# TIXhjq/ML_Function

Measured on AMD Instinct MI355X. Metric: samples/sec fwd+bwd xDeepFM-CIN B=4096,F=39,K=16, higher is better.
Workload: dtype f32

## Files before the change

ml_function_amd/csrc/cin.hip:

```cpp
#include "cin_kernels.h"
#include "cin_tail.h"
#include "cin_launch.h"
#include "cin_qtail.h"
#include "cin_qsplit.h"
#include "cin_qmerge.h"

#include <stdlib.h>

namespace fil {

struct CinShape {
  int B, F, K, L;
  int H[kCinMaxL];
  int Hp(int l) const { return l == 0 ? F : H[l - 1]; }
  int HS(int l) const { return 128 * cdiv(H[l], 128); }
  int xps(int l) const { return l == 0 ? F : HS(l - 1); }
  long M() const { return (long)B * K; }
  int JT() const { return cin_jt_of(F); }
  int HSmax() const {
    int h = 0;
    for (int l = 0; l < L; ++l) h = std::max(h, HS(l));
    return h;
  }
};

static int check_shape(const char* fn, int B, int F, int K, int L, const int* H, CinShape& s) {
  if (B < 0 || F < 1 || K < 1 || L < 1 || H == nullptr) return fail(FIL_ERR_ARG, "%s: bad shape B=%d F=%d K=%d L=%d", fn, B, F, K, L);
  if (L > kCinMaxL) return fail(FIL_ERR_UNSUPPORTED, "%s: L=%d > %d", fn, L, kCinMaxL);
  if (F > kCinMaxFields) return fail(FIL_ERR_UNSUPPORTED, "%s: F=%d > %d fields", fn, F, kCinMaxFields);
  if ((long)B * K > (1L << 28)) return fail(FIL_ERR_UNSUPPORTED, "%s: B*K = %ld rows > 2^28 (row-split byte offsets of the dW kernel are 32-bit)", fn, (long)B * K);
  s.B = B; s.F = F; s.K = K; s.L = L;
  for (int l = 0; l < L; ++l) {
    if (H[l] < 1) return fail(FIL_ERR_ARG, "%s: H[%d]=%d", fn, l, H[l]);
    if (H[l] > kCinMaxH) return fail(FIL_ERR_UNSUPPORTED, "%s: H[%d]=%d > %d feature maps", fn, l, H[l], kCinMaxH);
    s.H[l] = H[l];
  }
  return FIL_OK;
}

static int chunks_of(int H) { return cdiv(H, 128); }
static int env_int(const char* name, int dflt) {
  const char* v = getenv(name);
  return v != nullptr && *v != 0 ? atoi(v) : dflt;
}
struct Knobs {
  int mb, sym, dw_mb, dw_splits, dz_mb, tail_splits, tail_settle, tail_dz_mode, ksplit, dzs_mb, qtail, qmerge, dz2, fwdq, headfold, packfold, dwfold4;
};
static const Knobs& knobs() {
  static const Knobs k = {env_int("FIL_CIN_MB", 0), env_int("FIL_CIN_SYM", 1), env_int("FIL_CIN_DW_MB", 1), env_int("FIL_CIN_DW_SPLITS", 0),
                          env_int("FIL_CIN_DZ_MB", 1), env_int("FIL_CIN_TAIL_SPLITS", 0), env_int("FIL_CIN_TAIL_SETTLE", 0), env_int("FIL_CIN_TAIL_DZ_MODE", 0), env_int("FIL_CIN_KSPLIT", -1), env_int("FIL_CIN_DZS_MB", 0), env_int("FIL_CIN_QTAIL", 1), env_int("FIL_CIN_QMERGE", 1), env_int("FIL_CIN_DZ2", 1), env_int("FIL_CIN_FWDQ", 1), env_int("FIL_CIN_HEADFOLD", 1), env_int("FIL_CIN_PACKFOLD", 1), env_int("FIL_CIN_DWFOLD4", 1)};
  return k;
}
struct CinTune {
  int mb_forced;
  bool sym, no_ksplit;
  explicit CinTune(int mode)
      : mb_forced((mode & FIL_CIN_MB2) ? 2 : knobs().mb), sym(knobs().sym != 0 && !(mode & FIL_CIN_NOSYM)), no_ksplit((mode & FIL_CIN_NOKSPLIT) != 0) {}
  int mb_rows(long M) const {
    if (mb_forced == 1 || mb_forced == 2) return mb_forced;
    return cdiv((int)std::min<long>(M, 1L << 30), 64) >= 768 ? 2 : 1;
  }
  int ksplit(long M) const {
    if (knobs().ksplit == 0 || no_ksplit) return 1;
    if (mb_rows(M) != 1) return 1;
    if (knobs().ksplit == 4) return 4;
    return cdiv((int)std::min<long>(M, 1L << 30), 32) <= 512 ? 4 : 1;
  }
};

static const char* kFwdNames[kCinMaxL] = {"cin_fwd_l1", "cin_fwd_l2", "cin_fwd_l3", "cin_fwd_l4", "cin_fwd_l5", "cin_fwd_l6", "cin_fwd_l7", "cin_fwd_l8"};
static const char* kDwNames[kCinMaxL] = {"cin_bwd_dw_l1", "cin_bwd_dw_l2", "cin_bwd_dw_l3", "cin_bwd_dw_l4", "cin_bwd_dw_l5", "cin_bwd_dw_l6", "cin_bwd_dw_l7", "cin_bwd_dw_l8"};
static const char* kDzNames[kCinMaxL] = {"cin_bwd_dz_l1", "cin_bwd_dz_l2", "cin_bwd_dz_l3", "cin_bwd_dz_l4", "cin_bwd_dz_l5", "cin_bwd_dz_l6", "cin_bwd_dz_l7", "cin_bwd_dz_l8"};
static double gemm_flops(long M, int Hp, int F, int H) { return 2.0 * (double)M * Hp * F * H; }

struct DwPlan {
  int MB, blocks_x, splits, rows_per_split, chunks;
};
static int cu_count() {
  static const int n = [] {
    int dev = 0, v = 0;
    if (hipGetDevice(&dev) != hipSuccess || hipDeviceGetAttribute(&v, hipDeviceAttributeMultiprocessorCount, dev) != hipSuccess || v <= 0) v = 256;
    return v;
  }();
  return n;
}

static DwPlan dw_plan(long M, int C, int H) {
  DwPlan p;
  p.chunks = chunks_of(H);
  p.MB = knobs().dw_mb == 2 ? 2 : 1;
  const int waves_c = cdiv(C, 32 * p.MB);
  p.blocks_x = cdiv(waves_c, 4);
  const long tiles = (long)p.blocks_x * p.chunks;
  const long ncu = cu_count();
  const long unit = 2 * kDwDepth;
  auto rows_of = [&](int splits) { return std::max<long>(unit, ((M + splits - 1) / splits + unit - 1) / unit * unit); };
  int best = knobs().dw_splits;
  if (best <= 0) {
    static const double t_of[4] = {0.0, 1.05e-4, 1.39e-4, 1.96e-4};
    double best_ms = -1.0;
    for (int sp = (int)std::max<long>(1, (M + (1L << 20) - 1) >> 20); sp <= 256; ++sp) {
      const long rps = rows_of(sp);
      const long real = (M + rps - 1) / rps;
      if (real != sp && sp > 1) continue;
      long wgs = tiles * real;
      double per_row = 0.0;
      while (wgs > 0) {
        const long round = std::min(wgs, 3 * ncu);
        per_row += t_of[std::min<long>(3, (round + ncu - 1) / ncu)];
        wgs -= round;
      }
      const double ms = (double)rps * per_row * p.MB + (double)real * C * H * 4.0 / 6e9;
      if (best_ms < 0 || ms < best_ms) best = sp, best_ms = ms;
      if (rps == unit) break;
    }
  }
  best = std::min(std::max(best, 1), 256);
  const long rps = rows_of(best);
  p.rows_per_split = (int)rps;
  p.splits = (int)std::max<long>(1, (M + rps - 1) / rps);
  return p;
}

static int launch_dw3(hipStream_t st, const DwPlan& p, const float* gT, int HS, const float* xT, const float* xpT, int xps, float* part,
                      long M, int F, int Hp, int H, int symD = 0, int xtra = 0) {
  const int items = p.blocks_x * p.splits * p.chunks;
  const dim3 grid((items + 7) / 8 * 8);
#define FIL_DW3(MBV, ONES) \
  hipLaunchKernelGGL((cin_dw3_kernel<MBV, ONES>), grid, dim3(kCinThreads), 0, st, gT, HS, xT, xpT, xps, part, (int)M, F, Hp, H, p.rows_per_split, \
                     p.blocks_x, p.chunks, items, symD, xtra)
  if (xT == nullptr) {
    if (p.MB == 2) FIL_DW3(2, true); else FIL_DW3(1, true);
  } else {
    if (p.MB == 2) FIL_DW3(2, false); else FIL_DW3(1, false);
  }
#undef FIL_DW3
  return p.splits;
}

struct TailGeom {
  bool on = false;
  int p = 0;
  int NCB = 0, JP = 0, JT4 = 0, NQ = 0, JHp = 0;
  int Hpp = 0, Hq = 0, HL = 0, Cp = 0, C1 = 0;
  int periods = 0, tiles = 0;
  size_t uf_floats = 0, uz_floats = 0;
};
static TailGeom tail_geom(const CinShape& s) {
  TailGeom g;
  if (s.L < 3 || !cin_tail_supported(s.F)) return g;
  g.on = true;
  g.p = s.L - 2;
  g.NCB = cin_tail_ncb(s.F);
  g.JP = 16 * g.NCB;
  g.JT4 = cin_tail_jt4(s.F);
  g.NQ = cin_tail_nq(s.F);
  g.JHp = 4 * g.NQ;
  g.Hpp = s.H[g.p - 1];
  g.Hq = s.H[g.p];
  g.HL = s.H[s.L - 1];
  g.Cp = g.Hpp * s.F;
  g.C1 = g.Cp + 1;
  const int JT = s.JT();
  g.periods = cdiv(g.Hpp, cin_dz_h_per_period(JT));
  g.tiles = g.periods * cin_dz_tiles_per_period(JT) + 1;
  g.uf_floats = (size_t)g.Hpp * g.JT4 * 64 * g.NCB + (size_t)align_up(g.JP + 1, 64);
  g.uz_floats = (size_t)g.tiles * 64 * g.JHp;
  return g;
}
constexpr int kCinRetiredBits = 0;
static bool tail_used(const CinShape& s, int mode) {
  if ((mode & (FIL_CIN_GENERAL | FIL_CIN_NOTAIL)) != 0) return false;
  const TailGeom g = tail_geom(s);
  if (!g.on) return false;
  return (mode & FIL_CIN_TAIL_ALWAYS) != 0 || 4 * g.JP <= 3 * g.Hq;
}
static bool qtail_used(const CinShape& s, int mode, const CinTune& tune) {
  if (s.M() <= 16384 && (mode & FIL_CIN_TAIL_ALWAYS) == 0) return false;
  return tail_used(s, mode) && s.L == 3 && tune.sym && s.F >= 2 && s.F + 2 <= kQtConst && s.H[0] <= 128 && 3 * s.F + 1 <= s.HSmax() && (mode & FIL_CIN_NOQTAIL) == 0 &&
         knobs().qtail != 0;
}
static bool qmerge_used(const CinShape& s, int mode, const CinTune& tune) {
  return qtail_used(s, mode, tune) && 3 * s.F + 3 <= s.HSmax() && (mode & FIL_CIN_NOQMERGE) == 0 && knobs().qmerge != 0;
}
constexpr int kCinPrecBf16 = 1 << 20;
static int qsplit_planes(int mode) { return (mode & kCinPrecBf16) != 0 ? 1 : 3; }
static bool qsplit_fwd_menu(int JT) { return JT >= 2 && JT <= 12 && JT % 2 == 0; }
static bool qsplit_used(const CinShape& s, int mode, const CinTune& tune) {
  return (mode & (FIL_CIN_BF16X3 | kCinPrecBf16)) != 0 && qmerge_used(s, mode, tune) && knobs().fwdq != 0 && knobs().dz2 != 0 && s.HS(0) == 128 &&
         qsplit_fwd_menu(cin_jt_sym(s.F));
}
static size_t qsplit_wb_bytes(const CinShape& s) { return (size_t)cin_qs_steps(s.F, cin_jt_sym(s.F)) * kQsStageBytes; }
static size_t qsplit_wzb_bytes(const CinShape& s) {
  const int jts = cin_jt_sym(s.F);
  return ((size_t)cdiv(s.F, cin_dz_h_per_period(jts)) * cin_dz_tiles_per_period(jts) + 1) * 8 * 3072;
}
static size_t qtail_wz_floats(const CinShape& s) {
  const int jts = cin_jt_sym(s.F);
  return ((size_t)cdiv(s.F, cin_dz_h_per_period(jts)) * cin_dz_tiles_per_period(jts) + 1) * 32 * s.HS(0);
}
static size_t qtail_wsn_floats(const CinShape& s) { return (size_t)chunks_of(s.H[0]) * 2 * s.JT() * 128; }
static size_t qtail_saved_floats(const CinShape& s) {
  return (size_t)s.M() * s.HS(0) + (size_t)s.F * s.F * s.H[0] + (size_t)s.H[1] * s.F + 128 + (size_t)s.H[0] * s.F + qtail_wsn_floats(s) +
         qtail_wz_floats(s);
}
struct TailDwPlan {
  int blocks_x, splits, rows_per_split;
};
static TailDwPlan tail_dw_plan(long M, int C1) {
  TailDwPlan p;
  p.blocks_x = cdiv(C1, 16 * kTailCbw);
  const long unit = 4L * 4 * kTailDwDepth;
  long want = knobs().tail_splits > 0 ? knobs().tail_splits : std::max<long>(1, 2L * cu_count() / p.blocks_x);
  want = std::max<long>(want, (M + (1L << 22) - 1) >> 22);
  const long rows = std::max(unit, ((M + want - 1) / want + unit - 1) / unit * unit);
  p.rows_per_split = (int)rows;
  p.splits = (int)std::max<long>(1, (M + rows - 1) / rows);
  return p;
}

constexpr int kHeadChunk = 16;
constexpr int kColRows = 128;

static size_t saved_bytes(const CinShape& s) {
  size_t t = align_up((size_t)s.M() * s.F * sizeof(float), 256);
  for (int l = 0; l + 1 < s.L; ++l) t += align_up((size_t)s.M() * s.HS(l) * sizeof(float), 256);
  const TailGeom g = tail_geom(s);
  if (g.on) {
    size_t u = align_up((size_t)s.M() * s.F * sizeof(float), 256);
    for (int l = 0; l < g.p; ++l) u += align_up((size_t)s.M() * s.HS(l) * sizeof(float), 256);
    u += align_up((size_t)s.M() * g.JP * sizeof(float), 256) + align_up((g.uz_floats + g.uf_floats) * sizeof(float), 256) +
         align_up((size_t)g.Hq * s.F * sizeof(float), 256);
    t = std::max(t, u);
  }
  if (g.on && s.L == 3) {
    const size_t u = align_up((size_t)s.M() * s.F * sizeof(float), 256) + align_up((size_t)s.M() * s.HS(0) * sizeof(float), 256) +
                     align_up(qtail_saved_floats(s) * sizeof(float), 256);
    t = std::max(t, u);
  }
  return t;
}
static size_t wf_floats(const CinShape& s) {
  size_t w = 0;
  for (int l = 0; l < s.L; ++l) {
    w = std::max(w, (size_t)chunks_of(s.H[l]) * s.Hp(l) * 2 * s.JT() * 128);
  }
  w = std::max(w, (size_t)chunks_of(s.H[0]) * s.F * 2 * cin_jt_sym(s.F) * 128);
  w += (size_t)2 * 2 * s.JT() * 128;
  return w;
}
static int dz_periods(const CinShape& s, int l) { return cdiv(s.Hp(l), cin_dz_h_per_period(s.JT())); }
static size_t wz_floats(const CinShape& s) {
  const int jts = cin_jt_sym(s.F);
  size_t w = ((size_t)cdiv(s.F, cin_dz_h_per_period(jts)) * cin_dz_tiles_per_period(jts) + 1) * 32 * s.HS(0);
  w = std::max(w, (size_t)s.F * (s.F / 2 + 1) * s.H[0]);
  for (int l = 0; l < s.L; ++l) w = std::max(w, ((size_t)dz_periods(s, l) * cin_dz_tiles_per_period(s.JT()) + 1) * 32 * s.HS(l));
  return w;
}
static int pool_chunks(const CinShape& s, int l) { return std::max(chunks_of(s.H[l]), l > 0 ? chunks_of(s.H[l - 1]) : 1); }
static size_t fwd_ws_bytes(const CinShape& s) {
  size_t t = 0;
  for (int l = 0; l < s.L; ++l) t += align_up((size_t)pool_chunks(s, l) * s.M() * sizeof(float), 256);
  t += align_up((size_t)s.Hp(s.L - 1) * s.F * sizeof(float), 256);
  t += align_up(wf_floats(s) * sizeof(float), 256);
  t += align_up((size_t)kCinMaxH * sizeof(float), 256);
  t += align_up(cin_x2_floats(s.M(), cin_x2_len(s.F)) * sizeof(float), 256);
  t += align_up((size_t)chunks_of(s.H[0]) * s.F * 2 * cin_jt_sym(s.F) * 128 * sizeof(float), 256);
  t += align_up(qsplit_wb_bytes(s), 256);
  return t;
}
static size_t dw_part_floats(const CinShape& s) {
  size_t pmax = 0;
  for (int l = 0; l < s.L; ++l) pmax = std::max(pmax, (size_t)dw_plan(s.M(), s.Hp(l) * s.F, s.H[l]).splits * s.Hp(l) * s.F * s.H[l]);
  const int csym = s.F * (s.F / 2 + 1);
  pmax = std::max(pmax, (size_t)dw_plan(s.M(), csym, s.H[0]).splits * csym * s.H[0]);
  pmax = std::max(pmax, (size_t)dw_plan(s.M(), csym + s.F, s.H[0]).splits * (csym + s.F) * s.H[0]);
  if (s.L == 3) pmax = std::max(pmax, (size_t)cin_dwq_plan(s.M(), csym + s.F, cu_count()).pairs * (csym + s.F) * 256);
  if (s.L == 3) pmax = std::max(pmax, (size_t)cin_dwqb_plan(s.M(), csym + s.F, cu_count()).splits * (csym + s.F) * 256);
  pmax = std::max(pmax, (size_t)dw_plan(s.M(), s.Hp(s.L - 1), s.F).splits * s.Hp(s.L - 1) * s.F);
  pmax = std::max(pmax, (size_t)dw_plan(s.M(), s.F, s.Hp(s.L - 1)).splits * s.Hp(s.L - 1) * s.F);
  const TailGeom g = tail_geom(s);
  if (g.on) {
    pmax = std::max(pmax, (size_t)tail_dw_plan(s.M(), g.C1).splits * g.C1 * g.JP + (size_t)cdiv(g.Cp, kTailPc) * g.Hq * s.F);
  }
  return pmax;
}
static size_t bwd_ws_bytes(const CinShape& s) {
  const size_t LK = (size_t)s.L * s.K;
  const size_t M = (size_t)s.M();
  size_t t = 0;
  t += align_up((size_t)s.B * LK * sizeof(float), 256);
  t += 2 * align_up(M * s.HSmax() * sizeof(float), 256);
  t += align_up(dw_part_floats(s) * sizeof(float), 256);
  const size_t nblk = (size_t)cdiv(std::max(1, s.B), kHeadChunk);
  const size_t ncol = (M + kColRows - 1) / kColRows;
  t += align_up(std::max(ncol * s.HSmax(), nblk * (LK + 1)) * sizeof(float), 256);
  const size_t cl = (size_t)std::max(s.Hp(s.L - 1), s.L == 3 ? s.H[0] : 0) * s.F;
  t += 2 * align_up(cl * sizeof(float), 256);
  t += align_up(wz_floats(s) * sizeof(float), 256);
  t += 2 * align_up(M * s.F * sizeof(float), 256);
  t += align_up((size_t)s.F * s.F * kCinMaxH * sizeof(float), 256);
  t += align_up(((M + 255) / 256 + 1) * kQtConst * sizeof(float), 256);
  t += align_up(((M + 255) / 256) * (LK + 1) * sizeof(float), 256);
  t += 2 * align_up(qsplit_wzb_bytes(s), 256);
  return t;
}

template <typename KernelT>
static void allow_lds(KernelT kernel, size_t sh) {
  if (sh > 48 * 1024) (void)hipFuncSetAttribute(reinterpret_cast<const void*>(kernel), hipFuncAttributeMaxDynamicSharedMemorySize, (int)sh);
}

}

using namespace fil;

extern "C" size_t fil_cin_saved_bytes(int B, int F, int K, int L, const int* H) {
  CinShape s;
  if (check_shape("fil_cin_saved_bytes", B, F, K, L, H, s) != FIL_OK || B == 0) return 0;
  return saved_bytes(s);
}

extern "C" size_t fil_cin_fwd_workspace_bytes(int B, int F, int K, int L, const int* H) {
  CinShape s;
  if (check_shape("fil_cin_fwd_workspace_bytes", B, F, K, L, H, s) != FIL_OK || B == 0) return 0;
  return fwd_ws_bytes(s);
}

extern "C" size_t fil_cin_bwd_workspace_bytes(int B, int F, int K, int L, const int* H) {
  CinShape s;
  if (check_shape("fil_cin_bwd_workspace_bytes", B, F, K, L, H, s) != FIL_OK || B == 0) return 0;
  return bwd_ws_bytes(s);
}

extern "C" int fil_cin_grad_ready_points(int B, int F, int K, int L, const int* H, int mode, int* point) {
  CinShape s;
  if (int rc = check_shape("fil_cin_grad_ready_points", B, F, K, L, H, s)) return rc;
  if (point == nullptr || mode < 0 || mode > 1023) return fail(FIL_ERR_ARG, "fil_cin_grad_ready_points: point == NULL or mode %d out of range", mode);
  if ((mode & kCinRetiredBits) != 0) return fail(FIL_ERR_UNSUPPORTED, "fil_cin_grad_ready_points: mode %d holds a retired bit (2: the split-bf16 experiment)", mode);
  if (B == 0) {
    for (int i = 0; i <= L; ++i) point[i] = 0;
    return 1;
  }
  int pt = 0, l = L - 1;
  point[L] = pt++;
  if (qmerge_used(s, mode, CinTune(mode))) {
    point[0] = point[L] = 0;
    pt = 1;
    point[1] = point[2] = pt++;
    return pt;
  }
  if (tail_used(s, mode)) {
    point[L - 1] = point[L - 2] = pt++;
    l = L - 3;
  }
  for (; l >= 0; --l) point[l] = pt++;
  return pt;
}

#define FIL_CIN_CHECK_ARG(cond)                                                        \
  do {                                                                                 \
    if (!(cond)) return ::fil::fail(FIL_ERR_ARG, "%s: bad argument: %s", who, #cond); \
  } while (0)

static int cin_precision_bits(const char* who, int mode, int precision, int* bits) {
  if (precision != FIL_CIN_PREC_DEFAULT && precision != FIL_CIN_PREC_BF16)
    return fail(FIL_ERR_ARG, "%s: precision %d (0 DEFAULT, 1 BF16)", who, precision);
  if (precision == FIL_CIN_PREC_BF16 && (mode & FIL_CIN_BF16X3) != 0)
    return fail(FIL_ERR_ARG, "%s: precision BF16 with mode bit BF16X3 (mode %d): two operand precisions", who, mode);
  *bits = precision == FIL_CIN_PREC_BF16 ? kCinPrecBf16 : 0;
  return FIL_OK;
}

extern "C" int fil_cin_precision_used(int B, int F, int K, int L, const int* H, int mode, int precision) {
  CinShape s;
  if (int rc = check_shape("fil_cin_precision_used", B, F, K, L, H, s)) return rc;
  if (mode < 0 || mode > 1023 || (mode & kCinRetiredBits) != 0) return fail(FIL_ERR_UNSUPPORTED, "fil_cin_precision_used: mode %d", mode);
  int bits = 0;
  if (int rc = cin_precision_bits("fil_cin_precision_used", mode, precision, &bits)) return rc;
  if (bits == 0 || B == 0) return FIL_CIN_PREC_DEFAULT;
  return qsplit_used(s, mode | bits, CinTune(mode)) ? FIL_CIN_PREC_BF16 : FIL_CIN_PREC_DEFAULT;
}

static int cin_fwd_impl(const char* who, const float* x, const float* const* W, const float* const* bias, const float* dense_w,
                        const float* dense_b, float* out, float* pooled, float* saved, int B, int F, int K, int L,
                        const int* H, int output_dim, int mode, int precision, void* workspace, size_t workspace_bytes, void* stream) {
  CinShape s;
  int rc = check_shape(who, B, F, K, L, H, s);
  if (rc != FIL_OK) return rc;
  if (mode < 0 || mode > 1023 || (mode & kCinRetiredBits) != 0)
    return fail(FIL_ERR_UNSUPPORTED, "%s: mode %d (bits: 1 general kernels, 2 BF16X3, 4 MB2, 8 NOSYM, 16 X_TRANSPOSED, 32 NOTAIL, 64 TAIL_ALWAYS, 128 NOKSPLIT, 256 NOQTAIL, 512 NOQMERGE)", who, mode);
  {
    int bits = 0;
    if ((rc = cin_precision_bits(who, mode, precision, &bits)) != FIL_OK) return rc;
    mode |= bits;
  }
  const bool xt_in = (mode & FIL_CIN_X_TRANSPOSED) != 0;
  const CinTune tune(mode);
  const bool tail = tail_used(s, mode);
  const bool qtail = qtail_used(s, mode, tune);
  const bool qmerge = qmerge_used(s, mode, tune);
  const bool qsplit = qsplit_used(s, mode, tune);
  const int qnp = qsplit_planes(mode);
  const TailGeom tg = tail_geom(s);
  mode &= 1;
  if (B == 0) return FIL_OK;
  FIL_CIN_CHECK_ARG(x && W && bias && pooled && saved);
  FIL_CIN_CHECK_ARG(output_dim != 1 || (dense_w && dense_b && out));
  if (workspace == nullptr || workspace_bytes < fwd_ws_bytes(s))
    return fail(FIL_ERR_WORKSPACE, "fil_cin_fwd: workspace %zu < %zu bytes", workspace_bytes, fwd_ws_bytes(s));
  hipStream_t st = (hipStream_t)stream;
  const long M = s.M();
  const int JT = s.JT(), MB = tune.mb_rows(M);
  Carver ws(workspace);
  PoolArgs pa;
  for (int l = 0; l < L; ++l) {
    pa.part[l] = ws.take<float>((size_t)pool_chunks(s, l) * M);
    pa.chunks[l] = chunks_of(H[l]);
  }
  float* wsum = ws.take<float>((size_t)s.Hp(L - 1) * F);
  float* Wf = ws.take<float>(wf_floats(s));
  float* qt_zbias = ws.take<float>((size_t)kCinMaxH);
  const int XL = cin_x2_len(F);
  float* x2T = ws.take<float>(cin_x2_floats(M, XL));
  const bool need_x2 = tune.sym;
  float* WfT = ws.take<float>((size_t)chunks_of(H[0]) * F * 2 * cin_jt_sym(F) * 128);
  u32x4* Wb = reinterpret_cast<u32x4*>(ws.take<unsigned char>(qsplit_wb_bytes(s)));
  Carver sv(saved);
  float* xT_own = sv.take<float>((size_t)M * F);
  const float* xT = xt_in ? x : xT_own;
  float *tailY = nullptr, *tailUz = nullptr, *tailBmT = nullptr;
  float *qtR = nullptr, *qtT = nullptr, *qtWsumL = nullptr, *qtCvec = nullptr, *qtWsumP = nullptr, *qtWsnP = nullptr, *qtWzT = nullptr;
  if (qtail) {
    Carver pv(saved);
    (void)pv.take<float>((size_t)M * F);
    (void)pv.take<float>((size_t)M * s.HS(0));
    float* q = pv.take<float>(qtail_saved_floats(s));
    qtR = q;
    qtT = qtR + (size_t)M * s.HS(0);
    qtWsumL = qtT + (size_t)F * F * H[0];
    qtCvec = qtWsumL + (size_t)H[1] * F;
    qtWsumP = qtCvec + 128;
    qtWsnP = qtWsumP + (size_t)H[0] * F;
    qtWzT = qtWsnP + qtail_wsn_floats(s);
  } else if (tail) {
    Carver pv(saved);
    (void)pv.take<float>((size_t)M * F);
    for (int l = 0; l < tg.p; ++l) (void)pv.take<float>((size_t)M * s.HS(l));
    tailY = pv.take<float>((size_t)M * tg.JP);
    tailUz = pv.take<float>(tg.uz_floats + tg.uf_floats);
    tailBmT = pv.take<float>((size_t)tg.Hq * F);
  }
  const bool prep_fused = tail && tune.sym;
  if (qtail) {
    FIL_CIN_CHECK_ARG(W[0] && W[L - 1] && W[L - 2]);
    ProfScope ps("cin_fwd_prep", st, 2.0 * M * F * sizeof(float));
    const int JTs = cin_jt_sym(F), chunks0 = chunks_of(H[0]);
    const long npack = (long)chunks0 * F * 2 * JTs * 128;
    const bool fq = qmerge && knobs().fwdq != 0 && s.HS(0) == 128;
    const int nt = fq ? 0 : B, npk = (int)std::min<long>((npack + 255) / 256, 1024), nwl = cdiv(tg.Hq * F, 8), nwp = cdiv(tg.Hpp * F, 8);
    const size_t sh = (xt_in || fq) ? 0 : (size_t)F * (K + 1) * sizeof(float);
    allow_lds(cin_qtail_prep_kernel, sh);
    hipLaunchKernelGGL(cin_qtail_prep_kernel, dim3(nt + npk + nwl + nwp), dim3(256), sh, st, x, xT_own, F, K, nt, W[0], Wf, H[0], 2 * JTs, chunks0, npk,
                       W[L - 1], qtWsumL, tg.Hq, tg.HL, nwl, W[L - 2], qtWsumP, qtWsnP, tg.Hpp, 2 * JT, chunks_of(tg.Hpp), x2T, XL, xt_in ? 1 : 0);
  } else if (prep_fused) {
    FIL_CIN_CHECK_ARG(W[0] && W[L - 1]);
    ProfScope ps("cin_fwd_prep", st, 2.0 * M * F * sizeof(float));
    const int JTs = cin_jt_sym(F), chunks0 = chunks_of(H[0]);
    const long npack = (long)chunks0 * F * 2 * JTs * 128;
    const int nt = B, npk = (int)std::min<long>((npack + 255) / 256, 1024), nws = cdiv(tg.Hq * F, 8), nz = 64;
    const size_t sh = xt_in ? 0 : (size_t)F * (K + 1) * sizeof(float);
    allow_lds(cin_fwd_prep_kernel, sh);
    hipLaunchKernelGGL(cin_fwd_prep_kernel, dim3(nt + npk + nws + nz), dim3(256), sh, st, x, xT_own, F, K, nt, W[0], Wf, H[0], 2 * JTs, chunks0,
                       npk, W[L - 1], tailBmT, tg.Hq, tg.HL, nws, reinterpret_cast<float4*>(tailUz), (long)((tg.uz_floats + tg.uf_floats) / 4), x2T, XL,
                       xt_in ? 1 : 0);
  } else if (!xt_in || need_x2) {
    ProfScope ps("cin_transpose_in", st, 2.0 * M * F * sizeof(float));
    hipLaunchKernelGGL(cin_transpose_in_kernel, dim3(B), dim3(256), xt_in ? 0 : (size_t)F * (K + 1) * sizeof(float), st, x, xT_own, F, K,
                       need_x2 ? x2T : nullptr, XL, xt_in ? 1 : 0);
  }
  FIL_CHECK_LAUNCH();
  const float* xpT = xT;
  bool fused_last = false;
  bool head_done = false;
  for (int l = 0; l < L; ++l) {
    FIL_CIN_CHECK_ARG(W[l] && bias[l]);
    if (qtail && qmerge && l == 0 && knobs().fwdq != 0 && s.HS(0) == 128) {
      const int p = tg.p, lL = L - 1, Hpp = tg.Hpp, Hq = tg.Hq, HS0 = s.HS(0);
      FIL_CIN_CHECK_ARG(W[p] && W[lL] && bias[p] && bias[lL]);
      const int JTs = cin_jt_sym(F), chunks = chunks_of(Hpp);
      float* x1T = sv.take<float>((size_t)M * HS0);
      {
        ProfScope ps("cin_tail_prep", st);
        int ks = -1;
        if (!xt_in && K <= 64 && (K & (K - 1)) == 0 && (reinterpret_cast<uintptr_t>(x) & 15) == 0)
          for (ks = 0; (1 << ks) < K;) ++ks;
        const size_t sh_x = ks >= 0 ? (size_t)(64 >> ks) * F * (K + 1) : (xt_in ? (size_t)64 * (F | 1) : (size_t)F * (K + 1));
        const int tiles = cdiv(F, cin_dz_h_per_period(JTs)) * cin_dz_tiles_per_period(JTs) + 1;
        const bool fold = !qsplit && knobs().packfold != 0;
        const QtPackFold pf = fold ? QtPackFold{WfT, qtWzT, JTs, chunks, HS0, tiles} : QtPackFold{nullptr, nullptr, 0, 0, 0, 0};
        const size_t sh = std::max(cin_qtail_t_lds_floats(F, Hq, fold), sh_x) * sizeof(float);
        allow_lds(cin_qtail_t_x_kernel, sh);
        const int nx = (ks >= 0 || xt_in) ? (int)((M + 63) / 64) : B, nT = cin_qtail_t_wgs(Hpp);
        hipLaunchKernelGGL(cin_qtail_t_x_kernel, dim3(nT + nx), dim3(256), sh, st, W[p], qtWsumL, bias[p], bias[lL], tg.HL, qtT, qtCvec, qt_zbias, Hpp, F, Hq,
                           nT, x, xT_own, K, x2T, XL, xt_in ? 1 : 0, ks, (ks >= 0 || xt_in) ? (long)M : 0L, pf);
        if (!fold) {
          const long npack = (long)chunks * F * 2 * JTs * 128;
          const int nbf = (int)std::min<long>((npack + 255) / 256, 1024), nbz = (int)std::min<long>(((long)tiles * 32 * HS0 + 255) / 256, 1024);
          const int NTq = qsplit ? cin_qs_steps(F, JTs) : 0, nbq = qsplit ? std::min(cdiv(NTq * 512, 256), 512) : 0;
          if (qnp == 1)
            hipLaunchKernelGGL(cin_qtail_pack_kernel<1>, dim3(nbf + nbz + nbq), dim3(256), 0, st, qtT, WfT, qtWzT, F, Hpp, JTs, chunks, nbf, HS0, tiles, nbz,
                               W[0], H[0], Wb, NTq);
          else
            hipLaunchKernelGGL(cin_qtail_pack_kernel<3>, dim3(nbf + nbz + nbq), dim3(256), 0, st, qtT, WfT, qtWzT, F, Hpp, JTs, chunks, nbf, HS0, tiles, nbz,
                               W[0], H[0], Wb, NTq);
        }
      }
      FIL_CHECK_LAUNCH();
      {
        const double algo = gemm_flops(M, F, F, H[0]) + gemm_flops(M, Hpp, F, Hq) + gemm_flops(M, Hq, F, tg.HL);
        ProfScope ps("cin_fwd_q", st, algo, gemm_flops(M, 1, F * (F / 2 + 1), H[0]) + gemm_flops(M, 1, F * (F / 2 + 1), Hpp));
        CinHeadFold hf{};
        if (K <= 32 && (K & (K - 1)) == 0 && knobs().headfold != 0) {
          int ks = 0;
          while ((1 << ks) < K) ++ks;
          hf = CinHeadFold{pooled, output_dim == 1 ? out : nullptr, dense_w, dense_b, ks, (int)(L * K), p * K, lL * K};
          head_done = true;
        }
        if (qsplit) {
          const int NT = cin_qs_steps(F, JTs);
          if (!cin_launch_fwdq_b(st, qnp, JTs, x2T, XL, Wb, NT, bias[0], qtWsnP, JT, qtCvec, x1T, qtR, HS0, const_cast<float*>(pa.part[0]),
                                 const_cast<float*>(pa.part[p]), const_cast<float*>(pa.part[lL]), (int)M, F, H[0], hf))
            return fail(FIL_ERR_UNSUPPORTED, "fil_cin_fwd: no split-bf16 forward kernel for JT=%d (F=%d)", JTs, F);
        } else if (!cin_launch_fwdq(st, JTs, x2T, XL, Wf, WfT, bias[0], qtWsnP, JT, qtCvec, x1T, qtR, HS0, const_cast<float*>(pa.part[0]),
                                    const_cast<float*>(pa.part[p]), const_cast<float*>(pa.part[lL]), (int)M, F, H[0], hf))
          return fail(FIL_ERR_UNSUPPORTED, "fil_cin_fwd: no merged forward kernel for JT=%d (F=%d)", JTs, F);
        pa.chunks[0] = pa.chunks[p] = pa.chunks[lL] = 1;
      }
      FIL_CHECK_LAUNCH();
      break;
    }
    if (qtail && l == tg.p) {
      const int lL = L - 1, Hpp = tg.Hpp, Hq = tg.Hq, HS0 = s.HS(0);
      FIL_CIN_CHECK_ARG(W[lL] && bias[lL]);
      const int JTs = cin_jt_sym(F), chunks = chunks_of(Hpp);
      {
        ProfScope ps("cin_tail_prep", st);
        const size_t sh = cin_qtail_t_lds_floats(F, Hq, false) * sizeof(float);
        allow_lds(cin_qtail_t_kernel, sh);
        hipLaunchKernelGGL(cin_qtail_t_kernel, dim3(cin_qtail_t_wgs(Hpp)), dim3(256), sh, st, W[l], qtWsumL, bias[l], bias[lL], tg.HL, qtT, qtCvec, qt_zbias, Hpp, F, Hq);
        const long npack = (long)chunks * F * 2 * JTs * 128;
        const int tiles = cdiv(F, cin_dz_h_per_period(JTs)) * cin_dz_tiles_per_period(JTs) + 1;
        const int nbf = (int)std::min<long>((npack + 255) / 256, 1024), nbz = (int)std::min<long>(((long)tiles * 32 * HS0 + 255) / 256, 1024);
        hipLaunchKernelGGL(cin_qtail_pack_kernel<3>, dim3(nbf + nbz), dim3(256), 0, st, qtT, Wf, qtWzT, F, Hpp, JTs, chunks, nbf, HS0, tiles);
      }
      FIL_CHECK_LAUNCH();
      {
        const double algo = gemm_flops(M, Hpp, F, Hq) + gemm_flops(M, Hq, F, tg.HL);
        ProfScope ps("cin_fwd_tail", st, algo, gemm_flops(M, 1, F * (F / 2 + 1), Hpp));
        const int ks = tune.ksplit(M);
        cin_launch_fwd3_sym(st, MB, JTs, dim3(ks == 4 ? cdiv((int)M, 32) : cdiv((int)M, 128 * MB), chunks), xT, x2T, XL, Wf, qt_zbias, qtR, HS0,
                            const_cast<float*>(pa.part[lL]), (int)M, F, Hpp, ks);
      }
      FIL_CHECK_LAUNCH();
      {
        ProfScope ps("cin_tail_pool", st);
        const float* wsn = qtWsnP;
        float* pp = const_cast<float*>(pa.part[l]);
        float* pL = const_cast<float*>(pa.part[lL]);
        const dim3 grid((int)((M + 127) / 128));
#define FIL_QP(JTV) \
  case JTV: hipLaunchKernelGGL((cin_qtail_pool2_kernel<JTV>), grid, dim3(256), 0, st, xT, xpT, s.xps(l), wsn, qtR, HS0, qtCvec, pp, pL, (int)M, F, Hpp); break;
        switch (JT) { FIL_QP(4) FIL_QP(8) FIL_QP(12) FIL_QP(16) FIL_QP(20) FIL_QP(24) FIL_QP(28) FIL_QP(32) }
#undef FIL_QP
        pa.chunks[l] = pa.chunks[lL] = 1;
      }
      FIL_CHECK_LAUNCH();
      break;
    }
    if (tail && l == tg.p) {
      const int lL = L - 1;
      FIL_CIN_CHECK_ARG(W[lL] && bias[lL]);
      float* Y = tailY;
      float* Uz = tailUz;
      float* bmT = tailBmT;
      float* Uf = Uz + tg.uz_floats;
      float* consts = Uf + (size_t)tg.Hpp * tg.JT4 * 64 * tg.NCB;
      {
        ProfScope ps("cin_tail_prep", st);
        if (!prep_fused) {
          hipLaunchKernelGGL(cin_tail_wsum_kernel, dim3(cdiv(tg.Hq * F, 8)), dim3(256), 0, st, W[lL], bmT, tg.Hq, F, tg.HL);
          (void)hipMemsetAsync(Uz, 0, (tg.uz_floats + tg.uf_floats) * sizeof(float), st);
        }
        const size_t sh = (size_t)(F + 1) * (((tg.Hq + 3) & ~3) + 4) * sizeof(float);
        allow_lds(cin_tail_ueff_kernel, sh);
        hipLaunchKernelGGL(cin_tail_ueff_kernel, dim3(cdiv(tg.C1, kTailUc)), dim3(256), sh, st, W[l], bias[l], bmT, bias[lL], tg.HL, Uf, Uz, consts,
                           tg.Hpp, F, tg.Hq, tg.JT4, tg.JP, JT, tg.JHp);
      }
      FIL_CHECK_LAUNCH();
      {
        const double algo = gemm_flops(M, tg.Hpp, F, tg.Hq) + gemm_flops(M, tg.Hq, F, tg.HL);
        ProfScope ps("cin_fwd_tail", st, algo, 2.0 * (double)M * tg.Cp * (F + 1));
        const int RB = tune.mb_rows(M) == 2 ? 4 : 2;
        TailFwdArgs a{xT, xpT, s.xps(l), Uf, consts, Y, tg.JP, const_cast<float*>(pa.part[l]), const_cast<float*>(pa.part[lL]), (int)M, F, tg.Hpp,
                      tune.ksplit(M)};
        cin_launch_tail_fwd(st, RB, tg.JT4, tg.NCB, a);
        pa.chunks[l] = pa.chunks[lL] = 1;
      }
      FIL_CHECK_LAUNCH();
      break;
    }
    const int Hp = s.Hp(l), Hl = H[l], xps = s.xps(l);
    float* xoutT = l + 1 < L ? sv.take<float>((size_t)M * s.HS(l)) : nullptr;
    float* part = const_cast<float*>(pa.part[l]);
    const bool fuse_next = mode == 0 && l == L - 2 && !(l == 0 && tune.sym);
    if (l == L - 1 && mode == 0) {
      if (!fused_last) {
        const size_t sh = (size_t)Hp * ((F + 3) & ~3) * sizeof(float);
        ProfScope ps("cin_last_fwd", st, 2.0 * (double)M * Hp * F);
        hipLaunchKernelGGL(cin_wsum_kernel, dim3(cdiv(Hp * F, 8)), dim3(256), 0, st, W[l], wsum, Hp * F, Hl);
        allow_lds(cin_last_fwd_kernel, sh);
        hipLaunchKernelGGL(cin_last_fwd_kernel, dim3(cdiv((int)M, kLastRows)), dim3(256), sh, st, xT, xpT, xps, wsum, bias[l], part, (int)M, F, Hp, Hl);
        pa.chunks[l] = 1;
      }
    } else {
      const int chunks = chunks_of(Hl);
      if (l == 0 && tune.sym) {
        const int JTs = cin_jt_sym(F);
        const long npack = (long)chunks * F * 2 * JTs * 128;
        if (!prep_fused)
          hipLaunchKernelGGL(cin_pack_wf_sym_kernel, dim3((int)std::min<long>((npack + 255) / 256, 2048)), dim3(256), 0, st, W[l], Wf, F, Hl, 2 * JTs, chunks);
        ProfScope ps(kFwdNames[l], st, gemm_flops(M, Hp, F, Hl), gemm_flops(M, 1, F * (F / 2 + 1), Hl));
        const int ks = tune.ksplit(M);
        cin_launch_fwd3_sym(st, MB, JTs, dim3(ks == 4 ? cdiv((int)M, 32) : cdiv((int)M, 128 * MB), chunks), xT, x2T, XL, Wf, bias[l], xoutT, s.HS(l), part,
                            (int)M, F, Hl, ks);
      } else {
        const long npack = (long)chunks * Hp * 2 * JT * 128;
        hipLaunchKernelGGL(cin_pack_wf_kernel, dim3((int)std::min<long>((npack + 255) / 256, 2048)), dim3(256), 0, st, W[l], Wf, Hp, F, Hl, 2 * JT, chunks);
        const float* wsn = nullptr;
        if (fuse_next) {
          FIL_CIN_CHECK_ARG(W[l + 1] && bias[l + 1]);
          float* wsn_buf = Wf + (size_t)npack;
          hipLaunchKernelGGL(cin_wsum_wsn_kernel, dim3(cdiv(Hl * F, 8)), dim3(256), 0, st, W[l + 1], wsum, Hl * F, H[l + 1], wsn_buf, Hl, F, 2 * JT,
                             chunks);
          wsn = wsn_buf;
          pa.chunks[l + 1] = chunks;
          fused_last = true;
        }
        ProfScope ps(kFwdNames[l], st, gemm_flops(M, Hp, F, Hl) + (fuse_next ? 2.0 * (double)M * Hl * F : 0.0));
        cin_launch_fwd3(st, MB, JT, dim3(cdiv((int)M, 128 * MB), chunks), xT, xpT, xps, Wf, bias[l], xoutT, s.HS(l), part, (int)M, F, Hp, Hl,
                        wsn, fuse_next ? bias[l + 1] : nullptr, fuse_next ? H[l + 1] : 0, fuse_next ? const_cast<float*>(pa.part[l + 1]) : nullptr);
      }
    }
    FIL_CHECK_LAUNCH();
    xpT = xoutT;
  }
  if (!head_done) {
    ProfScope ps("cin_head_fwd", st);
    hipLaunchKernelGGL(cin_head_fwd_kernel, dim3(cdiv(B, kHeadSamples)), dim3(256), (size_t)kHeadSamples * L * K * sizeof(float), st, pa, dense_w, dense_b, pooled,
                       output_dim == 1 ? out : nullptr, B, K, L);
  }
  FIL_CHECK_LAUNCH();
  return FIL_OK;
}

extern "C" int fil_cin_fwd(const float* x, const float* const* W, const float* const* bias, const float* dense_w,
                           const float* dense_b, float* out, float* pooled, float* saved, int B, int F, int K, int L,
                           const int* H, int output_dim, int mode, void* workspace, size_t workspace_bytes, void* stream) {
  return cin_fwd_impl("fil_cin_fwd", x, W, bias, dense_w, dense_b, out, pooled, saved, B, F, K, L, H, output_dim, mode, FIL_CIN_PREC_DEFAULT, workspace,
                      workspace_bytes, stream);
}

extern "C" int fil_cin_fwd_p(const float* x, const float* const* W, const float* const* bias, const float* dense_w,
                             const float* dense_b, float* out, float* pooled, float* saved, int B, int F, int K, int L,
                             const int* H, int output_dim, int mode, int precision, void* workspace, size_t workspace_bytes, void* stream) {
  return cin_fwd_impl("fil_cin_fwd_p", x, W, bias, dense_w, dense_b, out, pooled, saved, B, F, K, L, H, output_dim, mode, precision, workspace,
                      workspace_bytes, stream);
}

static int cin_bwd_impl(const char* who, const float* x, const float* const* W, const float* const* bias, const float* dense_w,
                        const float* pooled, const float* saved, const float* g, float* dx, float* const* dW,
                        float* const* dbias, float* ddense_w, float* ddense_b, int B, int F, int K, int L, const int* H,
                        int output_dim, int mode, int precision, void* const* grad_ready_events, void* workspace, size_t workspace_bytes,
                        void* stream) {
  CinShape s;
  int rc = check_shape(who, B, F, K, L, H, s);
  if (rc != FIL_OK) return rc;
  if (mode < 0 || mode > 1023 || (mode & kCinRetiredBits) != 0)
    return fail(FIL_ERR_UNSUPPORTED, "%s: mode %d (bits: 1 general kernels, 2 BF16X3, 4 MB2, 8 NOSYM, 16 X_TRANSPOSED, 32 NOTAIL, 64 TAIL_ALWAYS, 128 NOKSPLIT, 256 NOQTAIL, 512 NOQMERGE)", who, mode);
  {
    int bits = 0;
    if ((rc = cin_precision_bits(who, mode, precision, &bits)) != FIL_OK) return rc;
    mode |= bits;
  }
  const bool xt_in = (mode & FIL_CIN_X_TRANSPOSED) != 0;
  const CinTune tune(mode);
  const bool tail = tail_used(s, mode);
  const bool qtail = qtail_used(s, mode, tune);
  const bool qmerge = qmerge_used(s, mode, tune);
  const bool qsplit = qsplit_used(s, mode, tune);
  const int qnp = qsplit_planes(mode);
  const TailGeom tg = tail_geom(s);
  mode &= 1;
  FIL_CIN_CHECK_ARG(W && dW && dbias);
  hipStream_t st = (hipStream_t)stream;
  const size_t LK = (size_t)L * K;
  auto ready = [&](int slot) {
    if (grad_ready_events != nullptr && grad_ready_events[slot] != nullptr) (void)hipEventRecord((hipEvent_t)grad_ready_events[slot], st);
  };
  if (B == 0) {
    for (int l = 0; l < L; ++l) {
      (void)hipMemsetAsync(dW[l], 0, (size_t)s.Hp(l) * F * H[l] * sizeof(float), st);
      (void)hipMemsetAsync(dbias[l], 0, (size_t)H[l] * sizeof(float), st);
    }
    if (output_dim == 1) {
      (void)hipMemsetAsync(ddense_w, 0, LK * sizeof(float), st);
      (void)hipMemsetAsync(ddense_b, 0, sizeof(float), st);
    }
    for (int l = 0; l <= L; ++l) ready(l);
    return FIL_OK;
  }
  FIL_CIN_CHECK_ARG(g && dx && saved && (x || !xt_in));
  FIL_CIN_CHECK_ARG(output_dim != 1 || (dense_w && pooled && ddense_w && ddense_b));
  if (workspace == nullptr || workspace_bytes < bwd_ws_bytes(s))
    return fail(FIL_ERR_WORKSPACE, "fil_cin_bwd: workspace %zu < %zu bytes", workspace_bytes, bwd_ws_bytes(s));
  const long M = s.M();
  const int JT = s.JT();
  Carver ws(workspace);
  float* dP = ws.take<float>((size_t)B * LK);
  float* Gbuf[2];
  Gbuf[0] = ws.take<float>((size_t)M * s.HSmax());
  Gbuf[1] = ws.take<float>((size_t)M * s.HSmax());
  float* part = ws.take<float>(dw_part_floats(s));
  const int nblk = cdiv(B, kHeadChunk);
  const int ncol = (int)((M + kColRows - 1) / kColRows);
  float* small = ws.take<float>(std::max((size_t)ncol * s.HSmax(), (size_t)nblk * (LK + 1)));
  const size_t cl = (size_t)s.Hp(L - 1) * F;
  const size_t cl_buf = (size_t)std::max(s.Hp(L - 1), L == 3 ? H[0] : 0) * F;
  float* wsum = ws.take<float>(cl_buf);
  float* vlast = ws.take<float>(cl_buf);
  float* Wz = ws.take<float>(wz_floats(s));
  float* dxT = ws.take<float>((size_t)M * F);
  float* gx0T = ws.take<float>((size_t)M * F);
  float* qt_dT = ws.take<float>((size_t)F * F * kCinMaxH);
  const int qt_ndc = (int)((M + 255) / 256);
  float* qt_dcpart = ws.take<float>((size_t)(qt_ndc + 1) * kQtConst);
  float* qt_hpart = ws.take<float>((size_t)qt_ndc * (LK + 1));
  u32x4* Wzb1 = reinterpret_cast<u32x4*>(ws.take<unsigned char>(qsplit_wzb_bytes(s)));
  u32x4* Wzb2 = reinterpret_cast<u32x4*>(ws.take<unsigned char>(qsplit_wzb_bytes(s)));

  Carver sv(const_cast<float*>(saved));
  const float* xT_own = sv.take<float>((size_t)M * F);
  const float* xT = xt_in ? x : xT_own;
  const float* maps[kCinMaxL];
  const float *tailY = nullptr, *tailUz = nullptr, *tailWsum = nullptr;
  const float *qtR = nullptr, *qtT = nullptr, *qtWsumL = nullptr, *qtCvec = nullptr, *qtWsumP = nullptr, *qtWsnP = nullptr, *qtWzT = nullptr;
  if (qtail) {
    maps[0] = sv.take<float>((size_t)M * s.HS(0));
    const float* q = sv.take<float>(qtail_saved_floats(s));
    qtR = q;
    qtT = qtR + (size_t)M * s.HS(0);
    qtWsumL = qtT + (size_t)F * F * H[0];
    qtCvec = qtWsumL + (size_t)H[1] * F;
    qtWsumP = qtCvec + 128;
    qtWsnP = qtWsumP + (size_t)H[0] * F;
    qtWzT = qtWsnP + qtail_wsn_floats(s);
  } else if (tail) {
    for (int l = 0; l < tg.p; ++l) maps[l] = sv.take<float>((size_t)M * s.HS(l));
    tailY = sv.take<float>((size_t)M * tg.JP);
    tailUz = sv.take<float>(tg.uz_floats + tg.uf_floats);
    tailWsum = sv.take<float>((size_t)tg.Hq * F);
  } else {
    for (int l = 0; l + 1 < L; ++l) maps[l] = sv.take<float>((size_t)M * s.HS(l));
  }

  const float* dPsrc = g;
  if (output_dim == 1 && qmerge) {
    dPsrc = dP;
  } else if (output_dim == 1) {
    ProfScope ps("cin_head_bwd", st);
    hipLaunchKernelGGL(cin_head_bwd_kernel, dim3(nblk), dim3(256), 0, st, g, dense_w, pooled, dP, small, B, (int)LK, kHeadChunk);
    if (!tail) hipLaunchKernelGGL(cin_reduce_kernel, dim3(cdiv((int)LK + 1, 64)), dim3(256), 0, st, small, ddense_w, (long)(LK + 1), nblk, ddense_b, (long)LK);
    FIL_CHECK_LAUNCH();
    dPsrc = dP;
  }
  if (!tail) ready(L);

  int cur = 0;
  int ltop = L - 1;
  bool dx_started = false;
  bool have_gx0 = false;
  bool wz_prepacked = false;
  bool qm_joined = false;
  if (qmerge) {
    const int p = tg.p, lL = L - 1, Hpp = tg.Hpp, Hq = tg.Hq, HS0 = s.HS(0);
    FIL_CIN_CHECK_ARG(bias && W[0] && W[p] && W[lL] && bias[p] && dW[0] && dW[p] && dW[lL] && dbias[0] && dbias[p] && dbias[lL]);
    const float* xpT = maps[p - 1];
    const int xps = s.xps(p);
    const float* dPp = dPsrc + (size_t)p * K;
    const float* dPL = dPsrc + (size_t)lL * K;
    const float* dPprev = dPsrc + (size_t)(p - 1) * K;
    const double algo_tail = gemm_flops(M, Hpp, F, Hq) + gemm_flops(M, Hq, F, tg.HL);
    const double algo1 = gemm_flops(M, F, F, H[0]);
    const int symD = F / 2 + 1, Cl = F * symD;
    const int JTs = cin_jt_sym(F);
    const int periods = cdiv(F, cin_dz_h_per_period(JTs));
    const int tiles0 = periods * cin_dz_tiles_per_period(JTs) + 1;
    const int XE = F + 3;
    float* xe = Gbuf[1];
    float* gxR = xe + (size_t)M * XE;
    float* dxR = gxR + (size_t)M * F;
    {
      ProfScope ps("cin_tail_a", st, (double)M * (2 * F + 3) * sizeof(float));
      const size_t sh = (size_t)256 * (F + 3 + (output_dim == 1 ? L : 0)) * sizeof(float);
      allow_lds(cin_qtail_xe_kernel<3>, sh);
      allow_lds(cin_qtail_xe_kernel<1>, sh);
      const int np = (int)std::min<long>(((long)tiles0 * 32 * HS0 + 255) / 256, 1024);
      const int nq2 = qsplit ? 2 * std::min(cdiv(tiles0 * 512, 256), 256) : 0;
      if (qnp == 1)
        hipLaunchKernelGGL(cin_qtail_xe_kernel<1>, dim3(qt_ndc + np + nq2), dim3(kXeThreads), sh, st, xT, dPL, dPp, (int)LK, K, xe, qt_dcpart, (int)M, F,
                           qt_ndc, output_dim == 1 ? g : nullptr, dense_w, pooled, dP, qt_hpart, (int)LK, lL, p, W[0], Wz, H[0], JTs, HS0, tiles0, np, qtT,
                           Hpp, Wzb1, Wzb2);
      else
        hipLaunchKernelGGL(cin_qtail_xe_kernel<3>, dim3(qt_ndc + np + nq2), dim3(kXeThreads), sh, st, xT, dPL, dPp, (int)LK, K, xe, qt_dcpart, (int)M, F,
                           qt_ndc, output_dim == 1 ? g : nullptr, dense_w, pooled, dP, qt_hpart, (int)LK, lL, p, W[0], Wz, H[0], JTs, HS0, tiles0, np, qtT,
                           Hpp, Wzb1, Wzb2);
    }
    FIL_CHECK_LAUNCH();
    {
      ProfScope ps("cin_last_bwd", st, 6.0 * (double)M * Hpp * F);
      cin_launch_last_bwd2(st, JT, xT, xpT, xps, qtWsumP, qtWsnP, dPp, (int)LK, dPprev, Gbuf[cur], HS0, dxT, (int)M, F, K, Hpp, qtR, HS0, dPL, small);
    }
    FIL_CHECK_LAUNCH();
    int dw_parts = 0;
    {
      ProfScope ps("cin_bwd_dw_q", st, algo1 + algo_tail, gemm_flops(M, 1, Cl, H[0]) + gemm_flops(M, 1, Cl, Hpp));
      if (qsplit) {
        const DwqbPlan bp = cin_dwqb_plan(M, Cl + F, cu_count());
        cin_launch_dwq_b(st, qnp, bp, Gbuf[cur], xpT, HS0, xe, XE, part, (int)M, F, symD);
        dw_parts = bp.splits;
      } else {
        const bool f4 = knobs().dwfold4 != 0;
        const DwqPlan dp = f4 ? cin_dwq_plan4(M, Cl + F, cu_count()) : cin_dwq_plan(M, Cl + F, cu_count());
        if (f4)
          hipLaunchKernelGGL((cin_dwq_kernel<kDwqDepth, 4>), dim3((dp.wgs + 7) / 8 * 8), dim3(kDwqThreads), 0, st, Gbuf[cur], xpT, HS0, xe, XE, part, (int)M, F,
                             symD, dp.rows_per_split, dp.splits, dp.ncol_full, dp.rem, dp.wgs_full, dp.wgs);
        else
          hipLaunchKernelGGL((cin_dwq_kernel<kDwqDepth, 2>), dim3((dp.wgs + 7) / 8 * 8), dim3(kDwqThreads), 0, st, Gbuf[cur], xpT, HS0, xe, XE, part, (int)M, F,
                             symD, dp.rows_per_split, dp.splits, dp.ncol_full, dp.rem, dp.wgs_full, dp.wgs);
        dw_parts = dp.pairs;
      }
    }
    FIL_CHECK_LAUNCH();
    {
      ProfScope ps("cin_reduce_dw", st);
      const int nb1 = cdiv(H[0], 64);
      const int nh = output_dim == 1 ? cdiv((int)LK + 1, 64) : 0;
      hipLaunchKernelGGL(cin_reduce_expand_q_kernel, dim3((Cl + F + 3) / 4 + nb1 + nh), dim3(256), 0, st, part, dw_parts, F, symD, H[0], Hpp, dW[0], qt_dT,
                         vlast, small, ncol, dbias[0], nb1, qt_hpart, qt_ndc, (int)LK, ddense_w, ddense_b);
    }
    FIL_CHECK_LAUNCH();
    ready(L);
    ready(0);
    {
      ProfScope ps("cin_tail_params", st);
      const size_t sh = cin_qtail_params_lds(F, Hq);
      allow_lds(cin_qtail_params_kernel, sh);
      float* dcfin = qt_dcpart + (size_t)qt_ndc * kQtConst;
      hipLaunchKernelGGL(cin_qtail_params_kernel, dim3(2 * Hpp + 1), dim3(256), sh, st, W[p], qtWsumL, qt_dT, vlast, dW[p], part, Hpp, F, Hq, qt_dcpart, qt_ndc,
                         dcfin);
      hipLaunchKernelGGL(cin_qtail_fill_kernel, dim3(cdiv(Hq * F, kQtFillCols)), dim3(kQtFillThreads), 0, st, part, Hpp, dcfin, bias[p], qtWsumL, dW[lL], dbias[p], dbias[lL], F, Hq,
                         tg.HL);
    }
    FIL_CHECK_LAUNCH();
    ready(lL);
    ready(p);
    const int NHMAX = HS0 / 2;
    if (NHMAX == 64 && knobs().dz2 != 0) {
      ProfScope ps("cin_bwd_dz_q", st, algo1 + algo_tail, gemm_flops(M, 1, Cl, H[0]) + gemm_flops(M, 1, Cl, Hpp));
      bool split_done = false;
      if (qsplit) {
        split_done = cin_launch_dz2_b(st, qnp, JTs, Gbuf[cur], xpT, HS0, dPL, (int)LK, K, Wzb1, Wzb2, xT, dxT, 1, (int)M, F, H[0], Hpp, periods, dx, qtCvec);
      }
      if (!split_done &&
          !cin_launch_dz2(st, JTs, Gbuf[cur], xpT, HS0, dPL, (int)LK, K, Wz, qtWzT, xT, dxT, 1, (int)M, F, H[0], Hpp, periods, dx, qtCvec))
        return fail(FIL_ERR_UNSUPPORTED, "fil_cin_bwd: no two-pass data-gradient kernel for JT=%d (F=%d)", JTs, F);
      qm_joined = true;
    } else {
      const bool two_waves = NHMAX == 64 && cin_dzs_two_waves(JTs) && tune.mb_forced != 2 && knobs().dzs_mb != 2;
      const int MBs = two_waves ? 1 : tune.mb_rows(M);
      const int ks = MBs != 1 ? 1 : tune.ksplit(M);
      const dim3 zgrid(ks == 4 ? cdiv((int)M, 32) : cdiv((int)M, 128 * MBs));
      {
        ProfScope ps("cin_bwd_dz_tail", st, algo_tail, gemm_flops(M, 1, Cl, Hpp));
        cin_launch_dz3_sym(st, MBs, JTs, NHMAX, zgrid, xpT, HS0, qtWzT, xT, gxR, dxR, 0, (int)M, F, Hpp, periods, ks);
      }
      FIL_CHECK_LAUNCH();
      {
        ProfScope ps("cin_bwd_dz_l1", st, algo1, gemm_flops(M, 1, Cl, H[0]));
        cin_launch_dz3_sym(st, MBs, JTs, NHMAX, zgrid, Gbuf[cur], HS0, Wz, xT, gx0T, dxT, 1, (int)M, F, H[0], periods, ks);
      }
      have_gx0 = true;
    }
    FIL_CHECK_LAUNCH();
    dx_started = true;
    ltop = -1;
  } else if (qtail) {
    const int p = tg.p, lL = L - 1, Hpp = tg.Hpp, Hq = tg.Hq, HS0 = s.HS(0);
    FIL_CIN_CHECK_ARG(bias && W[p] && W[lL] && bias[p] && dW[p] && dW[lL] && dbias[p] && dbias[lL]);
    const float* xpT = maps[p - 1];
    const int xps = s.xps(p);
    const float* dPp = dPsrc + (size_t)p * K;
    const float* dPL = dPsrc + (size_t)lL * K;
    const float* dPprev = dPsrc + (size_t)(p - 1) * K;
    const double algo = gemm_flops(M, Hpp, F, Hq) + gemm_flops(M, Hq, F, tg.HL);
    float* xs = Gbuf[1];
    float* gxR = xs + (size_t)M * (F + 1);
    float* dxR = gxR + (size_t)M * F;
    {
      ProfScope ps("cin_tail_a", st, (double)M * (F + 64) * sizeof(float));
      const size_t sh = (size_t)256 * (F + 3) * sizeof(float);
      allow_lds(cin_qtail_scale_kernel, sh);
      const int nh = output_dim == 1 ? cdiv((int)LK + 1, 64) : 0;
      FIL_CIN_CHECK_ARG(W[0]);
      const int JTs0 = cin_jt_sym(F);
      const int tiles0 = cdiv(F, cin_dz_h_per_period(JTs0)) * cin_dz_tiles_per_period(JTs0) + 1;
      const int np = (int)std::min<long>(((long)tiles0 * 32 * HS0 + 255) / 256, 1024);
      hipLaunchKernelGGL(cin_qtail_scale_kernel, dim3(qt_ndc + nh + np), dim3(256), sh, st, xT, dPL, dPp, (int)LK, K, xs, qt_dcpart, (int)M, F, qt_ndc, small,
                         ddense_w, ddense_b, (int)LK, nblk, nh, W[0], Wz, H[0], JTs0, HS0, tiles0);
      wz_prepacked = true;
    }
    FIL_CHECK_LAUNCH();
    ready(L);
    {
      ProfScope ps("cin_last_bwd", st, 6.0 * (double)M * Hpp * F);
      cin_launch_last_bwd2(st, JT, xT, xpT, xps, qtWsumP, qtWsnP, dPp, (int)LK, dPprev, Gbuf[cur], HS0, dxT, (int)M, F, K, Hpp, qtR, HS0, dPL, small);
    }
    FIL_CHECK_LAUNCH();
    const int symD = F / 2 + 1, Cl = F * symD;
    const int JTs = cin_jt_sym(F);
    {
      ProfScope ps("cin_bwd_dw_tail", st, algo, gemm_flops(M, 1, Cl, Hpp));
      const int parts = launch_dw3(st, dw_plan(M, Cl + F, Hpp), xpT, HS0, xT, xs, F + 1, part, M, F, F, Hpp, symD, F);
      const long nW = (long)Cl * Hpp, pstride = (long)(Cl + F) * Hpp;
      hipLaunchKernelGGL(cin_reduce_expand_sym_kernel, dim3((int)((nW + 63) / 64) + cdiv(F * Hpp, 64)), dim3(256), 0, st, part, qt_dT, F, symD, Hpp, parts,
                         pstride, vlast, (long)F * Hpp);
    }
    FIL_CHECK_LAUNCH();
    {
      ProfScope ps("cin_tail_params", st);
      const size_t sh = cin_qtail_params_lds(F, Hq);
      allow_lds(cin_qtail_params_kernel, sh);
      float* dcfin = qt_dcpart + (size_t)qt_ndc * kQtConst;
      hipLaunchKernelGGL(cin_qtail_params_kernel, dim3(2 * Hpp + 1), dim3(256), sh, st, W[p], qtWsumL, qt_dT, vlast, dW[p], part, Hpp, F, Hq, qt_dcpart, qt_ndc,
                         dcfin);
      hipLaunchKernelGGL(cin_qtail_fill_kernel, dim3(cdiv(Hq * F, kQtFillCols)), dim3(kQtFillThreads), 0, st, part, Hpp, dcfin, bias[p], qtWsumL, dW[lL], dbias[p], dbias[lL], F, Hq,
                         tg.HL);
    }
    FIL_CHECK_LAUNCH();
    ready(lL);
    ready(p);
    {
      const int periods = cdiv(F, cin_dz_h_per_period(JTs));
      ProfScope ps("cin_bwd_dz_tail", st, algo, gemm_flops(M, 1, Cl, Hpp));
      const int NHMAX = HS0 / 2;
      const bool two_waves = NHMAX == 64 && cin_dzs_two_waves(JTs) && tune.mb_forced != 2 && knobs().dzs_mb != 2;
      const int MBs = two_waves ? 1 : tune.mb_rows(M);
      const int ks = MBs != 1 ? 1 : tune.ksplit(M);
      cin_launch_dz3_sym(st, MBs, JTs, NHMAX, dim3(ks == 4 ? cdiv((int)M, 32) : cdiv((int)M, 128 * MBs)), xpT, HS0, qtWzT, xT, gxR, dxR, 0, (int)M, F, Hpp,
                         periods, ks);
    }
    FIL_CHECK_LAUNCH();
    dx_started = true;
    ltop = p - 1;
  } else if (tail) {
    const int p = tg.p, lL = L - 1;
    FIL_CIN_CHECK_ARG(bias && W[p] && W[lL] && bias[p] && dW[p] && dW[lL] && dbias[p] && dbias[lL]);
    const float* xpT = maps[p - 1];
    const int xps = s.xps(p);
    const double algo = gemm_flops(M, tg.Hpp, F, tg.Hq) + gemm_flops(M, tg.Hq, F, tg.HL);
    float* Apk = Gbuf[1];
    wz_prepacked = p == 1 && tune.sym && F >= 2;
    {
      ProfScope ps("cin_tail_a", st, (double)M * (F + 64) * sizeof(float));
      const int na = (int)std::min<long>((M * 16 * tg.NCB + 255) / 256, 4096);
      const int nh = output_dim == 1 ? cdiv((int)LK + 1, 64) : 0;
      int np = 0, JTs = 0, tiles0 = 0;
      if (wz_prepacked) {
        FIL_CIN_CHECK_ARG(W[0]);
        JTs = cin_jt_sym(F);
        tiles0 = cdiv(F, cin_dz_h_per_period(JTs)) * cin_dz_tiles_per_period(JTs) + 1;
        np = (int)std::min<long>(((long)tiles0 * 32 * s.HS(0) + 255) / 256, 1024);
      }
      hipLaunchKernelGGL(cin_tail_pre_kernel, dim3(na + nh + np), dim3(256), 0, st, xT, dPsrc, (int)LK, K, p, lL, Apk, (int)M, F, tg.NCB, na, small,
                         ddense_w, ddense_b, (int)LK, nblk, nh, W[0], Wz, H[0], JTs, s.HS(0), tiles0);
    }
    FIL_CHECK_LAUNCH();
    ready(L);
    const TailDwPlan tp = tail_dw_plan(M, tg.C1);
    {
      ProfScope ps("cin_bwd_dw_tail", st, algo, 2.0 * (double)M * tg.C1 * (F + 2));
      TailDwArgs a{Apk, xT, xpT, xps, part, (int)M, F, tg.Hpp, tg.JP, tp.rows_per_split, tp.blocks_x, tp.blocks_x * tp.splits, knobs().tail_settle != 0};
      cin_launch_tail_dw(st, tg.NCB, a);
    }
    FIL_CHECK_LAUNCH();
    {
      ProfScope ps("cin_tail_params", st);
      const int nblk_p = cdiv(tg.Cp, kTailPc);
      const int ldb = (tg.Hq + 3) & ~3;
      const size_t sh = ((size_t)(F + 1) * ldb + (size_t)tg.JP * (kTailPc + 4) + (size_t)kTailPc * ldb) * sizeof(float);
      allow_lds(cin_tail_params_kernel, sh);
      float* partB = part + (size_t)tp.splits * tg.C1 * tg.JP;
      float* qones = vlast;
      hipLaunchKernelGGL(cin_tail_params_kernel, dim3(2 * nblk_p), dim3(256), sh, st, part, tp.splits, W[p], tailWsum, dW[p], dbias[p], partB, qones,
                         tg.Cp, F, tg.Hq, tg.JP);
      hipLaunchKernelGGL(cin_tail_fill_kernel, dim3(cdiv(tg.Hq * F, 64)), dim3(256), 0, st, partB, nblk_p, qones, bias[p], dW[lL], dbias[lL], F,
                         tg.Hq, tg.HL);
    }
    FIL_CHECK_LAUNCH();
    ready(lL);
    ready(p);
    {
      ProfScope ps("cin_bwd_dz_tail", st, algo, 2.0 * (double)M * tg.Cp * (F + 1));
      TailDzArgs a{tailUz, xT, xpT, xps, tailY, tg.JP, dPsrc, (int)LK, K, p, lL, Gbuf[cur], s.HS(p - 1), dxT, (int)M, F, tg.Hpp, tg.periods, knobs().tail_dz_mode,
                   tune.ksplit(M)};
      cin_launch_tail_dz(st, JT, tg.NQ, a);
    }
    FIL_CHECK_LAUNCH();
    dx_started = true;
    ltop = p - 1;
  } else if (mode == 0) {
    const int l = L - 1;
    FIL_CIN_CHECK_ARG(W[l] && dW[l] && dbias[l]);
    const int Hp = s.Hp(l), Hl = H[l], xps = s.xps(l);
    const float* xpT = l == 0 ? xT : maps[l - 1];
    const float* dPl = dPsrc + (size_t)l * K;
    const float* dPprev = l > 0 ? dPsrc + (size_t)(l - 1) * K : nullptr;
    const size_t shw = (size_t)Hp * ((F + 3) & ~3) * sizeof(float);
    ProfScope ps("cin_last_bwd", st, 6.0 * (double)M * Hp * F);
    hipLaunchKernelGGL(cin_wsum_wsn_kernel, dim3(cdiv(Hp * F, 8)), dim3(256), 0, st, W[l], wsum, Hp * F, Hl, l > 0 ? Wz : nullptr, Hp, F, 2 * JT,
                       chunks_of(Hp));
    hipLaunchKernelGGL(cin_slice_sum_kernel, dim3(nblk), dim3(256), 0, st, dPl, (int)LK, small, B, K, kHeadChunk);
    {
      float* yT = Gbuf[1];
      const int YS = (F + 3) & ~3;
      const long tot = M * YS;
      hipLaunchKernelGGL(cin_scale_rows3_kernel, dim3((int)std::min<long>((tot + 255) / 256, 4096)), dim3(256), 0, st, xT, dPl, (int)LK, K, yT, (int)M, F, YS);
      const bool swap = l > 0;
      int nb;
      if (swap) nb = launch_dw3(st, dw_plan(M, F, Hp), xpT, xps, nullptr, yT, YS, part, M, 1, F, Hp);
      else nb = launch_dw3(st, dw_plan(M, Hp, F), yT, YS, nullptr, xpT, xps, part, M, 1, Hp, F);
      hipLaunchKernelGGL(cin_reduce_kernel, dim3(cdiv((int)cl, 64)), dim3(256), 0, st, part, vlast, (long)cl, nb);
      hipLaunchKernelGGL(cin_fill_rows_kernel, dim3((int)std::min<long>(((long)cl * Hl + 255) / 256, 2048)), dim3(256), 0, st, vlast, dW[l], (long)cl, Hl,
                         swap ? F : 0, Hp, small, nblk, dbias[l]);
    }
    ready(l);
    if (l > 0) {
      cin_launch_last_bwd2(st, JT, xT, xpT, xps, wsum, Wz, dPl, (int)LK, dPprev, Gbuf[cur], s.HS(l - 1), dxT, (int)M, F, K, Hp);
    } else {
      const size_t shb = shw + (size_t)kLastRows * (kLastFMax + 1) * sizeof(float);
      allow_lds(cin_last_bwd_kernel, shb);
      hipLaunchKernelGGL(cin_last_bwd_kernel, dim3(cdiv((int)M, kLastRows)), dim3(256), shb, st, xT, xpT, xps, wsum, dPl, (int)LK, dPprev,
                         nullptr, 0, dxT, 1, (int)M, F, K, Hp);
    }
    FIL_CHECK_LAUNCH();
    dx_started = true;
    ltop = L - 2;
  } else {
    const long total = M * s.HS(L - 1);
    ProfScope ps("cin_bcast_g", st, (double)total * sizeof(float));
    hipLaunchKernelGGL(cin_bcast3_kernel, dim3((int)std::min<long>((total + 255) / 256, 4096)), dim3(256), 0, st, dPsrc + (size_t)(L - 1) * K, (int)LK,
                       K, Gbuf[cur], s.HS(L - 1), (int)M, H[L - 1]);
    FIL_CHECK_LAUNCH();
  }
  for (int l = ltop; l >= 0; --l) {
    FIL_CIN_CHECK_ARG(W[l] && dW[l] && dbias[l]);
    const int Hp = s.Hp(l), Hl = H[l], HSl = s.HS(l), xps = s.xps(l);
    const float* xpT = l == 0 ? xT : maps[l - 1];
    const float* G = Gbuf[cur];
    {
      ProfScope ps("cin_dbias", st, (double)M * Hl * sizeof(float));
      if (!(qtail && l == ltop)) hipLaunchKernelGGL(cin_colsum3_kernel, dim3(ncol), dim3(256), 0, st, G, HSl, small, (int)M, Hl, kColRows);
      hipLaunchKernelGGL(cin_reduce_kernel, dim3(cdiv(Hl, 64)), dim3(256), 0, st, small, dbias[l], (long)Hl, ncol);
    }
    FIL_CHECK_LAUNCH();
    int parts;
    const int symD = (l == 0 && tune.sym) ? F / 2 + 1 : 0;
    const int Cl = symD > 0 ? F * symD : Hp * F;
    {
      ProfScope ps(kDwNames[l], st, gemm_flops(M, Hp, F, Hl), gemm_flops(M, 1, Cl, Hl));
      parts = launch_dw3(st, dw_plan(M, Cl, Hl), G, HSl, xT, xpT, xps, part, M, F, Hp, Hl, symD);
    }
    FIL_CHECK_LAUNCH();
    const long nW = (long)Cl * Hl;
    {
      ProfScope ps("cin_reduce_dw", st, (double)(parts + 1) * nW * sizeof(float));
      if (symD > 0) hipLaunchKernelGGL(cin_reduce_expand_sym_kernel, dim3((int)((nW + 63) / 64)), dim3(256), 0, st, part, dW[l], F, symD, Hl, parts);
      else hipLaunchKernelGGL(cin_reduce_kernel, dim3((int)((nW + 63) / 64)), dim3(256), 0, st, part, dW[l], nW, parts);
    }
    FIL_CHECK_LAUNCH();
    ready(l);
    {
      const int NHMAX = HSl / 2;
      const int MB = NHMAX == 128 ? 1 : tune.mb_rows(M);
      const int MBg = NHMAX == 128 ? 1 : ((knobs().dz_mb == 2 && JT <= 28) ? 2 : 1);
      const float* dPprev = l > 0 ? dPsrc + (size_t)(l - 1) * K : nullptr;
      if (l == 0 && tune.sym && F >= 2) {
        const int JTs = cin_jt_sym(F);
        const int periods = cdiv(F, cin_dz_h_per_period(JTs));
        const int tiles = periods * cin_dz_tiles_per_period(JTs) + 1;
        const long npack = (long)tiles * 32 * HSl;
        const bool two_waves = NHMAX == 64 && cin_dzs_two_waves(JTs) && tune.mb_forced != 2 && knobs().dzs_mb != 2;
        const int MBs = two_waves ? 1 : MB;
        if (!wz_prepacked) {
          hipLaunchKernelGGL(cin_pack_wz_sym_kernel, dim3((int)std::min<long>((npack + 255) / 256, 2048)), dim3(256), 0, st, W[l], Wz, F, Hl, JTs, HSl, tiles);
        }
        ProfScope ps(kDzNames[l], st, gemm_flops(M, Hp, F, Hl), gemm_flops(M, 1, F * (F / 2 + 1), Hl));
        const int ks = (NHMAX != 64 || MBs != 1) ? 1 : tune.ksplit(M);
        cin_launch_dz3_sym(st, MBs, JTs, NHMAX, dim3(ks == 4 ? cdiv((int)M, 32) : cdiv((int)M, 128 * MBs)), G, HSl, Wz, xT, gx0T, dxT,
                           dx_started ? 1 : 0, (int)M, F, Hl, periods, ks);
      } else {
        const int periods = dz_periods(s, l);
        const int tiles = periods * cin_dz_tiles_per_period(JT) + 1;
        const long npack = (long)tiles * 32 * HSl;
        hipLaunchKernelGGL(cin_pack_wz_kernel, dim3((int)std::min<long>((npack + 255) / 256, 2048)), dim3(256), 0, st, W[l], Wz, Hp, F, Hl, JT, HSl, tiles);
        ProfScope ps(kDzNames[l], st, gemm_flops(M, Hp, F, Hl));
        cin_launch_dz3(st, MBg, JT, NHMAX, dim3(cdiv((int)M, 128 * MBg)), G, HSl, Wz, xT, xpT, xps, dPprev, (int)LK, K,
                       l > 0 ? Gbuf[cur ^ 1] : nullptr, l > 0 ? s.HS(l - 1) : 0, l == 0 ? gx0T : nullptr, dxT, dx_started ? 1 : 0,
                       (int)M, F, Hp, Hl, periods);
      }
      dx_started = true;
      if (l == 0) have_gx0 = true;
    }
    FIL_CHECK_LAUNCH();
    cur ^= 1;
  }
  if (!qm_joined) {
    ProfScope ps("cin_transpose_out", st, 2.0 * M * F * sizeof(float));
    if (qmerge)
      hipLaunchKernelGGL(cin_transpose_out_kernel, dim3(B), dim3(256), (size_t)K * (F + 1) * sizeof(float), st, dxT, have_gx0 ? gx0T : nullptr, dx, F, K,
                         Gbuf[1] + (size_t)M * (F + 3), Gbuf[1] + (size_t)M * (F + 3) + (size_t)M * F, qtCvec, dPsrc + (size_t)(L - 1) * K, (int)LK);
    else if (qtail)
      hipLaunchKernelGGL(cin_transpose_out_kernel, dim3(B), dim3(256), (size_t)K * (F + 1) * sizeof(float), st, dxT, have_gx0 ? gx0T : nullptr, dx, F, K,
                         Gbuf[1] + (size_t)M * (F + 1), Gbuf[1] + (size_t)M * (F + 1) + (size_t)M * F, qtCvec, dPsrc + (size_t)(L - 1) * K, (int)LK);
    else
      hipLaunchKernelGGL(cin_transpose_out_kernel, dim3(B), dim3(256), (size_t)K * (F + 1) * sizeof(float), st, dxT, have_gx0 ? gx0T : nullptr, dx, F, K);
  }
  FIL_CHECK_LAUNCH();
  return FIL_OK;
}

extern "C" int fil_cin_bwd(const float* x, const float* const* W, const float* const* bias, const float* dense_w,
                           const float* pooled, const float* saved, const float* g, float* dx, float* const* dW,
                           float* const* dbias, float* ddense_w, float* ddense_b, int B, int F, int K, int L, const int* H,
                           int output_dim, int mode, void* const* grad_ready_events, void* workspace, size_t workspace_bytes,
                           void* stream) {
  return cin_bwd_impl("fil_cin_bwd", x, W, bias, dense_w, pooled, saved, g, dx, dW, dbias, ddense_w, ddense_b, B, F, K, L, H, output_dim, mode,
                      FIL_CIN_PREC_DEFAULT, grad_ready_events, workspace, workspace_bytes, stream);
}

extern "C" int fil_cin_bwd_p(const float* x, const float* const* W, const float* const* bias, const float* dense_w,
                             const float* pooled, const float* saved, const float* g, float* dx, float* const* dW,
                             float* const* dbias, float* ddense_w, float* ddense_b, int B, int F, int K, int L, const int* H,
                             int output_dim, int mode, int precision, void* const* grad_ready_events, void* workspace, size_t workspace_bytes,
                             void* stream) {
  return cin_bwd_impl("fil_cin_bwd_p", x, W, bias, dense_w, pooled, saved, g, dx, dW, dbias, ddense_w, ddense_b, B, F, K, L, H, output_dim, mode,
                      precision, grad_ready_events, workspace, workspace_bytes, stream);
}
```

ml_function_amd/csrc/cin_kernels.h:

```cpp
#pragma once
#include "common.h"

namespace fil {

constexpr int kCinThreads = 256;
constexpr int kCinMaxL = 8;
constexpr int kCinMaxH = 256;

__device__ __forceinline__ f32x16 mfma32(float a, float b, f32x16 c) {
  return __builtin_amdgcn_mfma_f32_32x32x2f32(a, b, c, 0, 0, 0);
}

__device__ __forceinline__ void settle(float& v) { asm volatile("" : "+v"(v)); }
typedef float f32x4s __attribute__((ext_vector_type(4)));
__device__ __forceinline__ void settle(f32x4s& v) { asm volatile("" : "+v"(v)); }

__device__ __forceinline__ __amdgpu_buffer_rsrc_t make_rsrc(const float* p, long bytes) {
  return __builtin_amdgcn_make_buffer_rsrc(const_cast<float*>(p), 0, (int)std::min<long>(bytes, 0x7fffffffL), 0x00020000);
}
__device__ __forceinline__ __amdgpu_buffer_rsrc_t make_rsrc_uniform(const float* p, long bytes) {
  const unsigned long a = reinterpret_cast<unsigned long>(p);
  const unsigned lo = __builtin_amdgcn_readfirstlane((unsigned)a), hi = __builtin_amdgcn_readfirstlane((unsigned)(a >> 32));
  const int n = __builtin_amdgcn_readfirstlane((int)std::min<long>(bytes, 0x7fffffffL));
  return __builtin_amdgcn_make_buffer_rsrc(reinterpret_cast<float*>(((unsigned long)hi << 32) | lo), 0, n, 0x00020000);
// ... 956 lines not shown
  const long total = (long)M * YS;
  for (long i = (long)blockIdx.x * blockDim.x + threadIdx.x; i < total; i += (long)gridDim.x * blockDim.x) {
    const long m = i / YS;
    const int f = (int)(i - m * YS);
    const long b = m / K;
    yT[i] = f < F ? xT[m * F + f] * dP[b * ldp + (m - b * K)] : 0.f;
  }
}

__device__ __forceinline__ void cin_reduce_body(const float* __restrict__ part, float* __restrict__ out, long n, int parts,
                                                float* __restrict__ out2, long n1, int bid, long pstride = 0) {
  __shared__ float red[4][64];
  const int lane = threadIdx.x & 63, wave = threadIdx.x >> 6;
  const long i = (long)bid * 64 + lane;
  const long ps = pstride > 0 ? pstride : n;
  float t0 = 0.f, t1 = 0.f, t2 = 0.f, t3 = 0.f;
  if (i < n) {
    int p = wave;
    for (; p + 60 < parts; p += 64) {
      float u[16];
#pragma unroll
      for (int e = 0; e < 16; ++e) u[e] = part[(long)(p + 4 * e) * ps + i];
#pragma unroll
      for (int e = 0; e < 16; e += 4) {
        t0 += u[e];
        t1 += u[e + 1];
        t2 += u[e + 2];
        t3 += u[e + 3];
      }
    }
    for (; p + 12 < parts; p += 16) {
      t0 += part[(long)p * ps + i];
      t1 += part[(long)(p + 4) * ps + i];
      t2 += part[(long)(p + 8) * ps + i];
      t3 += part[(long)(p + 12) * ps + i];
    }
    for (; p < parts; p += 4) t0 += part[(long)p * ps + i];
  }
  red[wave][lane] = (t0 + t1) + (t2 + t3);
  __syncthreads();
  if (wave == 0 && i < n) {
    const float v = (red[0][lane] + red[1][lane]) + (red[2][lane] + red[3][lane]);
    if (out2 != nullptr && i >= n1) out2[i - n1] = v;
    else out[i] = v;
  }
}
static __global__ __launch_bounds__(256) void cin_reduce_kernel(const float* __restrict__ part, float* __restrict__ out, long n,
                                                         int parts, float* __restrict__ out2 = nullptr, long n1 = 0, long pstride = 0) {
  cin_reduce_body(part, out, n, parts, out2, n1, blockIdx.x, pstride);
}

static __global__ __launch_bounds__(256) void cin_reduce_expand_sym_kernel(const float* __restrict__ part, float* __restrict__ dW, int F, int D,
                                                                    int H, int parts, long pstride = 0, float* __restrict__ vout = nullptr,
                                                                    long nv = 0) {
  if (vout != nullptr) {
    const long nbw = ((long)F * D * H + 63) / 64;
    if ((long)blockIdx.x >= nbw) {
      cin_reduce_body(part + (long)F * D * H, vout, nv, parts, nullptr, 0, (int)(blockIdx.x - nbw), pstride);
      return;
    }
  }
  __shared__ float red[4][64];
  const int lane = threadIdx.x & 63, wave = threadIdx.x >> 6;
  const long n = (long)F * D * H;
  const long ps = pstride > 0 ? pstride : n;
  const long i = (long)blockIdx.x * 64 + lane;
  float t0 = 0.f, t1 = 0.f, t2 = 0.f, t3 = 0.f;
  if (i < n) {
    int p = wave;
    for (; p + 60 < parts; p += 64) {
      float u[16];
#pragma unroll
      for (int e = 0; e < 16; ++e) u[e] = part[(long)(p + 4 * e) * ps + i];
#pragma unroll
      for (int e = 0; e < 16; e += 4) {
        t0 += u[e];
        t1 += u[e + 1];
        t2 += u[e + 2];
        t3 += u[e + 3];
      }
    }
    for (; p + 12 < parts; p += 16) {
      t0 += part[(long)p * ps + i];
      t1 += part[(long)(p + 4) * ps + i];
      t2 += part[(long)(p + 8) * ps + i];
      t3 += part[(long)(p + 12) * ps + i];
    }
    for (; p < parts; p += 4) t0 += part[(long)p * ps + i];
  }
  red[wave][lane] = (t0 + t1) + (t2 + t3);
  __syncthreads();
  if (wave == 0 && i < n) {
    const float v = (red[0][lane] + red[1][lane]) + (red[2][lane] + red[3][lane]);
    const int col = (int)(i % H);
    const int pair = (int)(i / H);
    const int h = pair / D, d = pair - h * D;
    const int f = (h + d) % F;
    dW[((long)h * F + f) * H + col] = v;
    if (d != 0 && 2 * d != F) dW[((long)f * F + h) * H + col] = v;
  }
}

static __global__ __launch_bounds__(256) void cin_slice_sum_kernel(const float* __restrict__ dP, int ldp, float* __restrict__ part, int B,
                                                            int K, int bchunk) {
  __shared__ float red[256];
  const int b_lo = blockIdx.x * bchunk, b_hi = min(B, b_lo + bchunk);
  float t = 0.f;
  const int total = (b_hi - b_lo) * K;
  for (int i = threadIdx.x; i < total; i += 256) {
    const int b = b_lo + i / K, k = i % K;
    t += dP[(long)b * ldp + k];
  }
  red[threadIdx.x] = t;
  __syncthreads();
  for (int s = 128; s > 0; s >>= 1) {
    if (threadIdx.x < s) red[threadIdx.x] += red[threadIdx.x + s];
    __syncthreads();
  }
  if (threadIdx.x == 0) part[blockIdx.x] = red[0];
}

constexpr int kLastFMax = 64;

static __global__ __launch_bounds__(256) void cin_wsum_kernel(const float* __restrict__ W, float* __restrict__ wsum, int C, int H) {
  const int row = blockIdx.x * 8 + (threadIdx.x >> 5), l = threadIdx.x & 31;
  float t = 0.f;
  if (row < C)
    for (int n = l; n < H; n += 32) t += W[(long)row * H + n];
  t = half_wave_sum(t);
  if (row < C && l == 0) wsum[row] = t;
}

static __global__ __launch_bounds__(256) void cin_wsum_wsn_kernel(const float* __restrict__ W, float* __restrict__ wsum, int C, int H,
                                                           float* __restrict__ wsn, int Hp, int F, int JT2, int chunks) {
  const int row = blockIdx.x * 8 + (threadIdx.x >> 5), l = threadIdx.x & 31;
  float t = 0.f;
  if (row < C)
    for (int n = l; n < H; n += 32) t += W[(long)row * H + n];
  t = half_wave_sum(t);
  if (row < C && l == 0) {
    wsum[row] = t;
    if (wsn != nullptr) {
      const int n = row / F, fp = row - n * F;
      wsn[(((n >> 7) * JT2) + fp) * 128 + (n & 127)] = t;
    }
  }
  if (wsn != nullptr) {
    const int total = chunks * JT2 * 128;
    for (int i = blockIdx.x * blockDim.x + threadIdx.x; i < total; i += gridDim.x * blockDim.x) {
      const int col = i & 127, fp = (i >> 7) % JT2, chunk = (i >> 7) / JT2;
      if (fp >= F || chunk * 128 + col >= Hp) wsn[i] = 0.f;
    }
  }
}

__device__ __forceinline__ void stage_wsum(const float* __restrict__ wsum, float* ws, int Hp, int F, int FP4) {
  for (int idx = threadIdx.x; idx < Hp * FP4; idx += blockDim.x) {
    const int h = idx / FP4, f = idx - h * FP4;
    ws[idx] = f < F ? wsum[h * F + f] : 0.f;
  }
}

constexpr int kLastRows = 64;

static __global__ __launch_bounds__(256) void cin_last_fwd_kernel(const float* __restrict__ xT, const float* __restrict__ xpT, int xps,
                                                           const float* __restrict__ wsum, const float* __restrict__ bias,
                                                           float* __restrict__ pool, int M, int F, int Hp, int H) {
  extern __shared__ __attribute__((aligned(16))) float smem[];
  const int FP4 = (F + 3) & ~3;
  stage_wsum(wsum, smem, Hp, F, FP4);
  float bsum = 0.f;
  for (int n = 0; n < H; ++n) bsum += bias[n];
  __syncthreads();
  const int lane = threadIdx.x & 63, wave = threadIdx.x >> 6;
  const int m = blockIdx.x * kLastRows + wave * 16 + (lane & 15), hq = lane >> 4;
  const bool valid = m < M;
  const long mm = valid ? m : 0;
  float xr[kLastFMax];
#pragma unroll
  for (int f = 0; f < kLastFMax; ++f) xr[f] = (valid && f < F) ? xT[mm * F + f] : 0.f;
  const float* xprow = xpT + mm * xps;
  float p = 0.f;
  for (int h = hq; h < Hp; h += 4) {
    const float4* wrow = reinterpret_cast<const float4*>(smem + h * FP4);
    float t = 0.f;
#pragma unroll
    for (int f4 = 0; f4 < kLastFMax / 4; ++f4) {
      if (4 * f4 < F) {
        const float4 w = wrow[f4];
        t = fmaf(xr[4 * f4], w.x, t);
        t = fmaf(xr[4 * f4 + 1], w.y, t);
        t = fmaf(xr[4 * f4 + 2], w.z, t);
        t = fmaf(xr[4 * f4 + 3], w.w, t);
      }
    }
    p = fmaf(valid ? xprow[h] : 0.f, t, p);
  }
  p += __shfl_xor(p, 16);
  p += __shfl_xor(p, 32);
  if (valid && hq == 0) pool[m] = p + bsum;
}

static __global__ __launch_bounds__(256) void cin_last_bwd_kernel(const float* __restrict__ xT, const float* __restrict__ xpT, int xps,
                                                           const float* __restrict__ wsum, const float* __restrict__ dP, int ldp,
                                                           const float* __restrict__ dPprev, float* __restrict__ GprevT, int HSp,
                                                           float* __restrict__ dxT, int layer1, int M, int F, int K, int Hp) {
  extern __shared__ __attribute__((aligned(16))) float smem[];
  const int FP4 = (F + 3) & ~3;
  float* ts = smem + Hp * FP4;
  stage_wsum(wsum, smem, Hp, F, FP4);
  __syncthreads();
  const int lane = threadIdx.x & 63, wave = threadIdx.x >> 6;
  const int rowl = wave * 16 + (lane & 15), hq = lane >> 4;
  const int m = blockIdx.x * kLastRows + rowl;
  const bool valid = m < M;
  const long mm = valid ? m : 0;
  const int b = (int)(mm / K), k = (int)(mm - (long)b * K);
  float xr[kLastFMax], u[kLastFMax];
#pragma unroll
  for (int f = 0; f < kLastFMax; ++f) {
    xr[f] = (valid && f < F) ? xT[mm * F + f] : 0.f;
    u[f] = 0.f;
  }
  const float dp = valid ? dP[(long)b * ldp + k] : 0.f;
  const float dpp = (valid && dPprev != nullptr) ? dPprev[(long)b * ldp + k] : 0.f;
  const float* xprow = xpT + mm * xps;
  for (int h = hq; h < Hp; h += 4) {
    const float4* wrow = reinterpret_cast<const float4*>(smem + h * FP4);
    const float xph = valid ? xprow[h] : 0.f;
    float t = 0.f;
#pragma unroll
    for (int f4 = 0; f4 < kLastFMax / 4; ++f4) {
      if (4 * f4 < F) {
        const float4 w = wrow[f4];
        t = fmaf(xr[4 * f4], w.x, t);
        t = fmaf(xr[4 * f4 + 1], w.y, t);
        t = fmaf(xr[4 * f4 + 2], w.z, t);
        t = fmaf(xr[4 * f4 + 3], w.w, t);
        u[4 * f4] = fmaf(xph, w.x, u[4 * f4]);
        u[4 * f4 + 1] = fmaf(xph, w.y, u[4 * f4 + 1]);
        u[4 * f4 + 2] = fmaf(xph, w.z, u[4 * f4 + 2]);
        u[4 * f4 + 3] = fmaf(xph, w.w, u[4 * f4 + 3]);
      }
    }
    if (layer1) ts[rowl * (kLastFMax + 1) + h] = t;
    else if (valid) GprevT[mm * HSp + h] = fmaf(dp, t, dpp);
  }
  if (layer1) __syncthreads();
#pragma unroll
  for (int f = 0; f < kLastFMax; ++f) {
    if (f < F) {
      float v = u[f];
      v += __shfl_xor(v, 16);
      v += __shfl_xor(v, 32);
      if (layer1) v += ts[rowl * (kLastFMax + 1) + f];
      if (valid && hq == 0) dxT[mm * F + f] = dp * v;
    }
  }
}

static __global__ __launch_bounds__(256) void cin_fill_rows_kernel(const float* __restrict__ v, float* __restrict__ dW, long C, int H, int Ft,
                                                            int Hp, const float* __restrict__ bpart = nullptr, int bparts = 0,
                                                            float* __restrict__ dbias = nullptr) {
  if (bpart != nullptr && blockIdx.x == 0) {
    __shared__ float red[256];
    float t = 0.f;
    for (int p = threadIdx.x; p < bparts; p += 256) t += bpart[p];
    red[threadIdx.x] = t;
    __syncthreads();
    for (int s = 128; s > 0; s >>= 1) {
      if (threadIdx.x < s) red[threadIdx.x] += red[threadIdx.x + s];
      __syncthreads();
    }
    const float tot = red[0];
    for (int n = threadIdx.x; n < H; n += 256) dbias[n] = tot;
  }
  const long total = C * H;
  for (long i = (long)blockIdx.x * blockDim.x + threadIdx.x; i < total; i += (long)gridDim.x * blockDim.x) {
    const long c = i / H;
    dW[i] = Ft > 0 ? v[(c % Ft) * Hp + c / Ft] : v[c];
  }
}

constexpr int kLast2Ld = 66;
constexpr int kLast2Stage = 32 * kLast2Ld;
template <int JT>
__global__ __launch_bounds__(256, 2) void cin_last_bwd2_kernel(const float* __restrict__ xT, const float* __restrict__ xpT, int xps,
                                                            const float* __restrict__ wsum, const float* __restrict__ wsn,
                                                            const float* __restrict__ dP, int ldp, const float* __restrict__ dPprev,
                                                            float* __restrict__ GprevT, int HSp, float* __restrict__ dxT, int M, int F,
                                                            int K, int Hp, const float* __restrict__ Radd = nullptr, int HSr = 0,
                                                            const float* __restrict__ dPadd = nullptr, float* __restrict__ colpart = nullptr) {
  __shared__ float colred[4][128];
  extern __shared__ __attribute__((aligned(16))) float smem[];
  for (int i = threadIdx.x; i < Hp * F; i += 256) smem[i] = wsum[i];
  __syncthreads();
  const int tid = threadIdx.x, lane = tid & 63, wave = tid >> 6;
  const int r = lane & 31, half = lane >> 5;
  const int wrow0 = (blockIdx.x * 4 + wave) * 32;
  if (wrow0 >= M && colpart == nullptr) return;
  const long mq = min(wrow0 + r, M - 1);
  float* stg = smem + ((Hp * F + 3) & ~3) + wave * kLast2Stage;
  const int nrow = min(32, M - wrow0);
  if (nrow > 0) {
    const float4* src = reinterpret_cast<const float4*>(xT + (long)wrow0 * F);
    const int n4 = nrow * F / 4, tail = nrow * F - 4 * n4;
    for (int i = lane; i < n4; i += 64) *reinterpret_cast<float4*>(stg + 4 * i) = src[i];
    if (lane < tail) stg[4 * n4 + lane] = xT[(long)wrow0 * F + 4 * n4 + lane];
  }
  __builtin_amdgcn_wave_barrier();
  float xr[JT];
  {
    const float* xrow = stg + min(r, max(nrow, 1) - 1) * F;
#pragma unroll
    for (int j = 0; j < JT; ++j) {
      const int f = 2 * j + half;
      xr[j] = (f < F && nrow > 0) ? xrow[min(f, F - 1)] : 0.f;
    }
  }
  __shared__ float dps[4][3][32];
  if (half == 0) {
    const int b = (int)(mq / K), k = (int)(mq - (long)b * K);
    dps[wave][0][r] = dP[(long)b * ldp + k];
    dps[wave][1][r] = dPprev != nullptr ? dPprev[(long)b * ldp + k] : 0.f;
    dps[wave][2][r] = Radd != nullptr ? dPadd[(long)b * ldp + k] : 0.f;
  }
  __builtin_amdgcn_wave_barrier();
  auto phase_t = [&]() {
  const int chunks = (Hp + 127) >> 7;
  for (int chunk = 0; chunk < chunks; ++chunk) {
    f32x16 t[4];
#pragma unroll
    for (int nb = 0; nb < 4; ++nb)
#pragma unroll
      for (int i = 0; i < 16; ++i) t[nb][i] = 0.f;
    const float4* wsb = reinterpret_cast<const float4*>(wsn + (long)chunk * (2 * JT) * 128) + (half * 32 + r);
    constexpr int QB = JT % 5 == 0 ? 5 : 4;
#pragma unroll
    for (int j0 = 0; j0 < JT; j0 += QB) {
      float4 wq[QB];
#pragma unroll
      for (int j = 0; j < QB; ++j) wq[j] = wsb[(long)(2 * (j0 + j)) * 32];
      __builtin_amdgcn_sched_barrier(0);
#pragma unroll
      for (int j = 0; j < QB; ++j) {
        const float4 w = wq[j];
        t[0] = mfma32(xr[j0 + j], w.x, t[0]);
        t[1] = mfma32(xr[j0 + j], w.y, t[1]);
        t[2] = mfma32(xr[j0 + j], w.z, t[2]);
        t[3] = mfma32(xr[j0 + j], w.w, t[3]);
      }
    }
    const int n0 = chunk * 128 + 4 * r;
    float c0 = 0.f, c1 = 0.f, c2 = 0.f, c3 = 0.f;
    float4 rq[8];
#pragma unroll
    for (int reg = 0; reg < 16; ++reg) {
      if (Radd != nullptr && (reg & 7) == 0) {
#pragma unroll
        for (int u = 0; u < 8; ++u) {
          const long mm = min(wrow0 + mfma32_row(reg + u, half), M - 1);
          rq[u] = *reinterpret_cast<const float4*>(Radd + mm * HSr + n0);
        }
      }
      const int row = mfma32_row(reg, half);
      const int m = wrow0 + row;
      const float dpr = dps[wave][0][row], dppr = dps[wave][1][row], dpa = dps[wave][2][row];
      if (m < M) {
        float* dst = GprevT + (long)m * HSp + n0;
        float v0 = fmaf(dpr, t[0][reg], dppr), v1 = fmaf(dpr, t[1][reg], dppr);
        float v2 = fmaf(dpr, t[2][reg], dppr), v3 = fmaf(dpr, t[3][reg], dppr);
        if (Radd != nullptr) {
          const float4 ra = rq[reg & 7];
          v0 = fmaf(dpa, ra.x, v0);
          v1 = fmaf(dpa, ra.y, v1);
          v2 = fmaf(dpa, ra.z, v2);
          v3 = fmaf(dpa, ra.w, v3);
        }
        c0 += v0;
        c1 += v1;
        c2 += v2;
        c3 += v3;
        if (n0 + 3 < Hp) {
          *reinterpret_cast<float4*>(dst) = make_float4(v0, v1, v2, v3);
        } else {
          if (n0 < Hp) dst[0] = v0;
          if (n0 + 1 < Hp) dst[1] = v1;
          if (n0 + 2 < Hp) dst[2] = v2;
        }
      }
    }
    if (colpart != nullptr) {
      c0 = lane_halves_sum(c0);
      c1 = lane_halves_sum(c1);
      c2 = lane_halves_sum(c2);
      c3 = lane_halves_sum(c3);
      if (half == 0) *reinterpret_cast<float4*>(&colred[wave][4 * r]) = make_float4(c0, c1, c2, c3);
      __syncthreads();
      for (int n = tid; n < 128; n += 256)
        if (chunk * 128 + n < Hp) colpart[(long)blockIdx.x * Hp + chunk * 128 + n] = (colred[0][n] + colred[1][n]) + (colred[2][n] + colred[3][n]);
      __syncthreads();
    }
  }
  };
  auto phase_u = [&]() {
  if (wrow0 >= M) return;
  f32x16 u0, u1;
#pragma unroll
  for (int i = 0; i < 16; ++i) u0[i] = u1[i] = 0.f;
  const bool two = F > 32;
  const int quads = (Hp + 3) >> 2;
#pragma unroll 1
  for (int q0 = 0; q0 < quads; q0 += 16) {
    __builtin_amdgcn_wave_barrier();
    {
      float4 v[8];
#pragma unroll
      for (int i = 0; i < 8; ++i) {
        const int row = (lane >> 4) + 4 * i, c4 = lane & 15;
        const long mm = min(wrow0 + row, M - 1);
        v[i] = 4 * q0 + 4 * c4 < xps ? *reinterpret_cast<const float4*>(xpT + mm * xps + 4 * q0 + 4 * c4) : make_float4(0.f, 0.f, 0.f, 0.f);
      }
#pragma unroll
      for (int i = 0; i < 8; ++i) {
        const int row = (lane >> 4) + 4 * i, c4 = lane & 15;
        float* d = stg + row * kLast2Ld + 4 * c4;
        *reinterpret_cast<float2*>(d) = make_float2(v[i].x, v[i].y);
        *reinterpret_cast<float2*>(d + 2) = make_float2(v[i].z, v[i].w);
      }
    }
    __builtin_amdgcn_wave_barrier();
    float2 av[16];
    const float* xprow = stg + r * kLast2Ld + 2 * half;
#pragma unroll
    for (int i = 0; i < 16; ++i) av[i] = q0 + i < quads ? *reinterpret_cast<const float2*>(xprow + 4 * i) : make_float2(0.f, 0.f);
#pragma unroll
    for (int i0 = 0; i0 < 16; i0 += 4) {
      float b0[4][2], b1[4][2];
#pragma unroll
      for (int ii = 0; ii < 4; ++ii) {
        const int h = 4 * (q0 + i0 + ii) + 2 * half;
        const float* w0 = smem + min(h, Hp - 1) * F;
        const float* w1 = smem + min(h + 1, Hp - 1) * F;
        const int k0 = (h < Hp && r < F) ? -1 : 0, k1 = (h + 1 < Hp && r < F) ? -1 : 0;
        b0[ii][0] = __builtin_bit_cast(float, __builtin_bit_cast(int, w0[min(r, F - 1)]) & k0);
        b0[ii][1] = __builtin_bit_cast(float, __builtin_bit_cast(int, w1[min(r, F - 1)]) & k1);
        b1[ii][0] = b1[ii][1] = 0.f;
        if (two) {
          const int k2 = (h < Hp && r + 32 < F) ? -1 : 0, k3 = (h + 1 < Hp && r + 32 < F) ? -1 : 0;
          b1[ii][0] = __builtin_bit_cast(float, __builtin_bit_cast(int, w0[min(r + 32, F - 1)]) & k2);
          b1[ii][1] = __builtin_bit_cast(float, __builtin_bit_cast(int, w1[min(r + 32, F - 1)]) & k3);
        }
      }
      __builtin_amdgcn_sched_barrier(0);
#pragma unroll
      for (int ii = 0; ii < 4; ++ii) {
        u0 = mfma32(av[i0 + ii].x, b0[ii][0], u0);
        u0 = mfma32(av[i0 + ii].y, b0[ii][1], u0);
        if (two) {
          u1 = mfma32(av[i0 + ii].x, b1[ii][0], u1);
          u1 = mfma32(av[i0 + ii].y, b1[ii][1], u1);
        }
      }
    }
  }
#pragma unroll
  for (int reg = 0; reg < 16; ++reg) {
    const int m = wrow0 + mfma32_row(reg, half);
    if (m < M) {
      const float dpr = dps[wave][0][mfma32_row(reg, half)];
      if (r < F) dxT[(long)m * F + r] = dpr * u0[reg];
      if (two && r + 32 < F) dxT[(long)m * F + 32 + r] = dpr * u1[reg];
    }
  }
  };
  if ((blockIdx.x >> 3) & 1) {
    phase_u();
    phase_t();
  } else {
    phase_t();
    phase_u();
  }
}

struct PoolArgs {
  const float* part[kCinMaxL];
  int chunks[kCinMaxL];
};

constexpr int kHeadSamples = 8;
static __global__ __launch_bounds__(256) void cin_head_fwd_kernel(PoolArgs pa, const float* __restrict__ dense_w,
                                                           const float* __restrict__ dense_b, float* __restrict__ pooled,
                                                           float* __restrict__ out, int B, int K, int L) {
  extern __shared__ float sh[];
  const int LK = L * K;
  const long M = (long)B * K;
  const int b0 = blockIdx.x * kHeadSamples;
  const int nb = min(kHeadSamples, B - b0);
  for (int e = threadIdx.x; e < nb * LK; e += 256) {
    const int bl = e / LK, j = e - bl * LK;
    const int l = j / K, k = j - l * K;
    const long b = b0 + bl;
    float v = 0.f;
    for (int ch = 0; ch < pa.chunks[l]; ++ch) v += pa.part[l][(long)ch * M + b * K + k];
    pooled[b * LK + j] = v;
    if (out != nullptr) sh[e] = v * dense_w[j];
  }
  if (out == nullptr) return;
  __syncthreads();
  if (threadIdx.x < nb) {
    float o = 0.f;
    for (int j = 0; j < LK; ++j) o += sh[threadIdx.x * LK + j];
    out[b0 + threadIdx.x] = o + dense_b[0];
  }
}

static __global__ __launch_bounds__(256) void cin_head_bwd_kernel(const float* __restrict__ g, const float* __restrict__ dense_w,
                                                           const float* __restrict__ pooled, float* __restrict__ dP,
                                                           float* __restrict__ part, int B, int LK, int bchunk) {
  __shared__ float red[4][256];
  const int b_lo = blockIdx.x * bchunk, b_hi = min(B, b_lo + bchunk);
  if (LK + 1 <= 64) {
    const int j = threadIdx.x & 63, w = threadIdx.x >> 6;
    float t = 0.f;
    if (j <= LK) {
      const float wj = j < LK ? dense_w[j] : 0.f;
      for (int b = b_lo + w; b < b_hi; b += 4) {
        const float gb = g[b];
        if (j < LK) {
          dP[(long)b * LK + j] = gb * wj;
          t = fmaf(gb, pooled[(long)b * LK + j], t);
        } else {
          t += gb;
        }
      }
    }
    red[w][j] = t;
    __syncthreads();
    if (w == 0 && j <= LK) part[(long)blockIdx.x * (LK + 1) + j] = ((red[0][j] + red[1][j]) + red[2][j]) + red[3][j];
  } else {
    for (int j = threadIdx.x; j <= LK; j += 256) {
      const float wj = j < LK ? dense_w[j] : 0.f;
      float t = 0.f;
      for (int b = b_lo; b < b_hi; ++b) {
        const float gb = g[b];
        if (j < LK) {
          dP[(long)b * LK + j] = gb * wj;
          t = fmaf(gb, pooled[(long)b * LK + j], t);
        } else {
          t += gb;
        }
      }
      part[(long)blockIdx.x * (LK + 1) + j] = t;
    }
  }
}


}
```

ml_function_amd/csrc/cin_qmerge.h:

```cpp
#pragma once
#include "cin_kernels.h"
#include "cin_launch.h"
#include "cin_qtail.h"

namespace fil {

constexpr int kDwqDepth = 6;
constexpr int kDwqThreads = 512;
struct DwqPlan {
  int tiles, ncol_full, rem, splits, pairs, rows_per_split, wgs_full, wgs;
};
inline int cin_dwq_rem_wgs(int rem, int pairs) { return rem == 0 ? 0 : (rem == 1 ? (pairs + 3) / 4 : (rem == 2 ? (pairs + 1) / 2 : pairs)); }
inline DwqPlan cin_dwq_plan(long M, int C, int cus) {
  DwqPlan p;
  p.tiles = (C + 31) / 32;
  p.ncol_full = p.tiles / 4;
  p.rem = p.tiles % 4;
  const long unit = 2 * kDwqDepth;
  const long slots = cus;
  int best = 1;
  for (int s = 1; s <= 512; ++s) {
    if ((long)p.ncol_full * s + cin_dwq_rem_wgs(p.rem, s) > slots) break;
    best = s;
  }
  long want = std::max<long>(2L * best, (M + (1L << 20) - 1) >> 20);
  long rows = std::max(unit, ((M + want - 1) / want + unit - 1) / unit * unit);
  p.rows_per_split = (int)rows;
  p.splits = (int)std::max<long>(1, (M + rows - 1) / rows);
  p.pairs = (p.splits + 1) / 2;
  p.wgs_full = p.ncol_full * p.pairs;
  p.wgs = p.wgs_full + cin_dwq_rem_wgs(p.rem, p.pairs);
  return p;
}

inline DwqPlan cin_dwq_plan4(long M, int C, int cus) {
  DwqPlan p;
  p.tiles = (C + 31) / 32;
  p.ncol_full = p.tiles / 2;
  p.rem = p.tiles % 2;
  const long unit = 2 * kDwqDepth;
  int best = 1;
  for (int q = 1; q <= 256; ++q) {
    if ((long)p.ncol_full * q + (p.rem ? (q + 1) / 2 : 0) > cus) break;
    best = q;
  }
  long want = std::max<long>(4L * best, (M + (1L << 20) - 1) >> 20);
  long rows = std::max(unit, ((M + want - 1) / want + unit - 1) / unit * unit);
  p.rows_per_split = (int)rows;
  p.splits = (int)std::max<long>(1, (M + rows - 1) / rows);
  p.pairs = (p.splits + 3) / 4;
  p.wgs_full = p.ncol_full * p.pairs;
  p.wgs = p.wgs_full + (p.rem ? (p.pairs + 1) / 2 : 0);
  return p;
}

template <int DEPTH = kDwqDepth, int FOLD = 2>
__global__ __launch_bounds__(kDwqThreads, 2) void cin_dwq_kernel(const float* __restrict__ gT, const float* __restrict__ x1T, int HS, const float* __restrict__ xe,
                                                                int XE, float* __restrict__ part, int M, int F, int symD, int rows_per_split, int splits,
                                                                int ncol_full, int rem, int wgs_full, int wgs) {
  __shared__ float fold[4][128][64];
  const int tid = threadIdx.x, lane = tid & 63, wave = tid >> 6;
  const int r = lane & 31, half = lane >> 5;
  const int Cp = F * symD, C = Cp + F;
  const int item = (blockIdx.x & 7) * (gridDim.x >> 3) + (blockIdx.x >> 3);
  if (item >= wgs) return;
  const int wl = FOLD == 4 ? (wave & 1) : (wave & 3), up = FOLD == 4 ? (wave >> 1) : (wave >> 2);
  int tile, pair;
  bool idle = false;
  if constexpr (FOLD == 4) {
    if (item < wgs_full) {
      tile = (item % ncol_full) * 2 + wl;
      pair = item / ncol_full;
    } else {
      tile = ncol_full * 2;
      pair = 2 * (item - wgs_full) + wl;
    }
  } else if (item < wgs_full) {
    tile = (item % ncol_full) * 4 + wl;
    pair = item / ncol_full;
  } else {
    const int j = item - wgs_full;
    if (rem == 1) {
      tile = ncol_full * 4;
      pair = 4 * j + wl;
    } else if (rem == 2) {
      tile = ncol_full * 4 + (wl & 1);
      pair = 2 * j + (wl >> 1);
    } else {
      tile = ncol_full * 4 + wl;
      pair = j;
      idle = wl == 3;
    }
  }
  tile = __builtin_amdgcn_readfirstlane(tile);
  pair = __builtin_amdgcn_readfirstlane(pair);
  const int split = FOLD * pair + up;
  const int npairs = (splits + FOLD - 1) / FOLD;
  const int c0 = tile * 32;
  const int m_lo = split * rows_per_split;
  const int m_hi = min(M, m_lo + rows_per_split);
  const bool work = !idle && pair < npairs && split < splits && m_lo < m_hi;
  const long mrem = work ? (long)m_hi - m_lo : 0;
  const long mbase = work ? m_lo : 0;
  const __amdgpu_buffer_rsrc_t rg = make_rsrc_uniform(gT + mbase * HS, mrem * HS * 4);
  const __amdgpu_buffer_rsrc_t r1 = make_rsrc_uniform(x1T + mbase * HS, mrem * HS * 4);
  const __amdgpu_buffer_rsrc_t rx = make_rsrc_uniform(xe + mbase * XE, mrem * XE * 4);
  const int c = c0 + r;
  const int cc = c < C ? c : C - 1;
  int hh, ff, sel;
  if (cc < Cp) {
    hh = cc / symD;
    ff = (hh + (cc - hh * symD)) % F;
    sel = 0;
  } else {
    hh = F;
    ff = cc - Cp;
    sel = 1;
  }
  const int ho = (half * XE + hh) * 4, fo = (half * XE + ff) * 4, so = (half * XE + F + 1 + sel) * 4;
  const int go = (half * HS + 4 * r) * 4;
  const int steps = work ? (m_hi - m_lo + 1) >> 1 : 0;
  const int groups = (steps + DEPTH - 1) / DEPTH;

  f32x16 acc[8];
#pragma unroll
  for (int nb = 0; nb < 8; ++nb)
#pragma unroll
    for (int i = 0; i < 16; ++i) acc[nb][i] = 0.f;
  f32x4s qg[DEPTH], q1[DEPTH];
  float qh[DEPTH], qf[DEPTH], qs[DEPTH];
  auto fetch = [&](int s, int d) {
    const int row = 2 * s;
    qg[d] = __builtin_bit_cast(f32x4s, __builtin_amdgcn_raw_buffer_load_b128(rg, go, row * HS * 4, 0));
    q1[d] = __builtin_bit_cast(f32x4s, __builtin_amdgcn_raw_buffer_load_b128(r1, go, row * HS * 4, 0));
    qh[d] = __builtin_bit_cast(float, __builtin_amdgcn_raw_buffer_load_b32(rx, ho, row * XE * 4, 0));
    qf[d] = __builtin_bit_cast(float, __builtin_amdgcn_raw_buffer_load_b32(rx, fo, row * XE * 4, 0));
    qs[d] = __builtin_bit_cast(float, __builtin_amdgcn_raw_buffer_load_b32(rx, so, row * XE * 4, 0));
  };
#pragma unroll
  for (int d = 0; d < DEPTH; ++d) fetch(d, d);
  float ac = qh[0] * qf[0], ac2 = ac * qs[0], an, an2;
#pragma unroll 1
  for (int g = 0; g < groups; ++g) {
#pragma unroll
    for (int d = 0; d < DEPTH; ++d) {
      const f32x4s g4 = qg[d], x4 = q1[d];
      an = qh[(d + 1) % DEPTH] * qf[(d + 1) % DEPTH];
      an2 = an * qs[(d + 1) % DEPTH];
      __builtin_amdgcn_sched_barrier(0);
      acc[0] = mfma32(ac, g4[0], acc[0]);
      acc[1] = mfma32(ac, g4[1], acc[1]);
      acc[2] = mfma32(ac, g4[2], acc[2]);
      acc[3] = mfma32(ac, g4[3], acc[3]);
      acc[4] = mfma32(ac2, x4[0], acc[4]);
      acc[5] = mfma32(ac2, x4[1], acc[5]);
      acc[6] = mfma32(ac2, x4[2], acc[6]);
      acc[7] = mfma32(ac2, x4[3], acc[7]);
      ac = an;
      ac2 = an2;
      __builtin_amdgcn_sched_barrier(0);
      fetch(g * DEPTH + d + DEPTH, d);
      __builtin_amdgcn_sched_barrier(0);
    }
  }
  if constexpr (FOLD == 4) {
    const int slot = (up >> 1) * 2 + wl;
    if (up & 1) {
#pragma unroll
      for (int nb = 0; nb < 8; ++nb)
#pragma unroll
        for (int i = 0; i < 16; ++i) fold[slot][nb * 16 + i][lane] = acc[nb][i];
    }
    __syncthreads();
    if (!(up & 1)) {
#pragma unroll
      for (int nb = 0; nb < 8; ++nb)
#pragma unroll
        for (int i = 0; i < 16; ++i) acc[nb][i] += fold[slot][nb * 16 + i][lane];
    }
    __syncthreads();
    if (up == 2) {
#pragma unroll
      for (int nb = 0; nb < 8; ++nb)
#pragma unroll
        for (int i = 0; i < 16; ++i) fold[wl][nb * 16 + i][lane] = acc[nb][i];
    }
    __syncthreads();
    if (up != 0 || pair >= npairs) return;
#pragma unroll
    for (int nb = 0; nb < 8; ++nb)
#pragma unroll
      for (int i = 0; i < 16; ++i) acc[nb][i] += fold[wl][nb * 16 + i][lane];
  } else {
    if (up == 1) {
#pragma unroll
      for (int nb = 0; nb < 8; ++nb)
#pragma unroll
        for (int i = 0; i < 16; ++i) fold[wl][nb * 16 + i][lane] = acc[nb][i];
    }
    __syncthreads();
    if (up == 1 || idle || pair >= npairs) return;
#pragma unroll
    for (int nb = 0; nb < 8; ++nb)
#pragma unroll
      for (int i = 0; i < 16; ++i) acc[nb][i] += fold[wl][nb * 16 + i][lane];
  }
  float* pout = part + (long)pair * C * 256;
#pragma unroll
  for (int reg = 0; reg < 16; ++reg) {
    const int cr = c0 + mfma32_row(reg, half);
    if (cr < C) {
      float* dst = pout + (long)cr * 256 + 4 * r;
      if (cr < Cp) *reinterpret_cast<float4*>(dst) = make_float4(acc[0][reg], acc[1][reg], acc[2][reg], acc[3][reg]);
      *reinterpret_cast<float4*>(dst + 128) = make_float4(acc[4][reg], acc[5][reg], acc[6][reg], acc[7][reg]);
    }
  }
}

static __global__ __launch_bounds__(256) void cin_reduce_expand_q_kernel(const float* __restrict__ part, int parts, int F, int D, int H1, int H2,
                                                                          float* __restrict__ dW1, float* __restrict__ dT, float* __restrict__ vT,
                                                                          const float* __restrict__ bpart, int nbp, float* __restrict__ dbias1,
                                                                          int nb1, const float* __restrict__ hpart, int nhp, int LK,
                                                                          float* __restrict__ ddw, float* __restrict__ ddb) {
  const int Cp = F * D, C = Cp + F;
  const int nbw = (C + 3) / 4;
  if ((int)blockIdx.x >= nbw + nb1) {
    cin_reduce_body(hpart, ddw, (long)LK + 1, nhp, ddb, (long)LK, (int)blockIdx.x - nbw - nb1);
    return;
  }
  if ((int)blockIdx.x >= nbw) {
    cin_reduce_body(bpart, dbias1, (long)H1, nbp, nullptr, 0, (int)blockIdx.x - nbw);
    return;
  }
  const int lane = threadIdx.x & 63, wave = threadIdx.x >> 6;
  const int c = blockIdx.x * 4 + wave;
  if (c >= C) return;
  const long ps = (long)C * 256;
  const float* p0 = part + (long)c * 256 + 4 * lane;
  f32x4 t[8];
#pragma unroll
  for (int u = 0; u < 8; ++u) t[u] = f32x4{0.f, 0.f, 0.f, 0.f};
  int p = 0;
  for (; p + 7 < parts; p += 8) {
#pragma unroll
    for (int u = 0; u < 8; ++u) t[u] += *reinterpret_cast<const f32x4*>(p0 + (long)(p + u) * ps);
  }
  for (; p < parts; ++p) t[0] += *reinterpret_cast<const f32x4*>(p0 + (long)p * ps);
  const f32x4 v = ((t[0] + t[1]) + (t[2] + t[3])) + ((t[4] + t[5]) + (t[6] + t[7]));
  const int col = 4 * lane, n0 = col & 127;
  const bool second = col >= 128;
  const int H = second ? H2 : H1;
  if (c >= Cp) {
    if (second) {
#pragma unroll
      for (int e = 0; e < 4; ++e)
        if (n0 + e < H2) vT[(long)(c - Cp) * H2 + n0 + e] = v[e];
    }
    return;
  }
  const int h = c / D, d = c - h * D;
  const int f = (h + d) % F;
  float* dst = second ? dT : dW1;
  const bool twin = d != 0 && 2 * d != F;
  float* r0 = dst + ((long)h * F + f) * H + n0;
  float* r1 = dst + ((long)f * F + h) * H + n0;
  if ((H & 3) == 0 && n0 + 3 < H) {
    *reinterpret_cast<f32x4*>(r0) = v;
    if (twin) *reinterpret_cast<f32x4*>(r1) = v;
  } else {
#pragma unroll
    for (int e = 0; e < 4; ++e)
      if (n0 + e < H) {
        r0[e] = v[e];
        if (twin) r1[e] = v[e];
      }
  }
}

constexpr int kXeThreads = 1024;
template <int NP = 3>
static __global__ __launch_bounds__(kXeThreads) void cin_qtail_xe_kernel(const float* __restrict__ xT, const float* __restrict__ dPL,
                                                                  const float* __restrict__ dPp, int ldp, int K, float* __restrict__ xe,
                                                                  float* __restrict__ dcpart, int M, int F, int nscale,
                                                                  const float* __restrict__ g, const float* __restrict__ dense_w,
                                                                  const float* __restrict__ pooled, float* __restrict__ dP, float* __restrict__ hpart,
                                                                  int LK, int lL, int lp, const float* __restrict__ W0, float* __restrict__ Wz,
                                                                  int H0, int JTs, int HS0, int tiles0, int npz = -1,
                                                                  const float* __restrict__ Tq = nullptr, int HT = 0, u32x4* __restrict__ Wzb1 = nullptr,
                                                                  u32x4* __restrict__ Wzb2 = nullptr) {
  extern __shared__ __attribute__((aligned(16))) float smem[];
  if ((int)blockIdx.x >= nscale) {
    if (threadIdx.x >= 256) return;
    if (npz < 0) npz = gridDim.x - nscale;
    const int b = blockIdx.x - nscale;
    if (b < npz) cin_pack_wz_sym_body(W0, Wz, F, H0, JTs, HS0, tiles0, b, npz);
    else {
      const int nq = ((int)gridDim.x - nscale - npz) >> 1, q = b - npz;
      if (q < nq) cin_qs_pack_wz_body<NP>(W0, H0, Wzb1, tiles0, F, JTs, q, nq);
      else if (q < 2 * nq) cin_qs_pack_wz_body<NP>(Tq, HT, Wzb2, tiles0, F, JTs, q - nq, nq);
    }
    return;
  }
  const int nl = g != nullptr ? LK / K : 0;
  const int hl = nl + 1, XE = F + 3;
  const int tid = threadIdx.x;
  const long m0 = (long)blockIdx.x * 256;
  const int nrows = (int)min((long)256, (long)M - m0);
  float* xs = smem;
  float* dls = xs + 256 * F;
  float* dps = dls + 256;
  float* hd = dps + 256;
  {
    const float* src = xT + m0 * F;
    const int n = nrows * F;
    if ((reinterpret_cast<uintptr_t>(xT) & 15) == 0) {
      const int n4 = n >> 2;
      for (int i0 = tid; i0 < n4; i0 += 4 * kXeThreads) {
        float4 v[4];
#pragma unroll
        for (int u = 0; u < 4; ++u) v[u] = i0 + u * kXeThreads < n4 ? reinterpret_cast<const float4*>(src)[i0 + u * kXeThreads] : make_float4(0.f, 0.f, 0.f, 0.f);
#pragma unroll
        for (int u = 0; u < 4; ++u)
          if (i0 + u * kXeThreads < n4) reinterpret_cast<float4*>(xs)[i0 + u * kXeThreads] = v[u];
      }
      for (int i = 4 * n4 + tid; i < n; i += kXeThreads) xs[i] = src[i];
    } else {
      for (int i = tid; i < n; i += kXeThreads) xs[i] = src[i];
    }
    for (int i = n + tid; i < 256 * F; i += kXeThreads) xs[i] = 0.f;
  }
  if (tid < 256) {
    const long m = m0 + tid;
    float dl = 0.f, dp = 0.f;
    if (m < M) {
      const long b = m / K;
      const int k = (int)(m - b * K);
      if (g != nullptr) {
        const float gb = g[b];
        for (int l = 0; l < nl; ++l) {
          const float d = gb * dense_w[l * K + k];
          dP[b * LK + l * K + k] = d;
          hd[tid * hl + l] = gb * pooled[b * LK + l * K + k];
        }
        hd[tid * hl + nl] = k == 0 ? gb : 0.f;
        dl = gb * dense_w[lL * K + k];
        dp = gb * dense_w[lp * K + k];
      } else {
        dl = dPL[b * ldp + k];
        dp = dPp[b * ldp + k];
      }
    } else if (g != nullptr) {
      for (int l = 0; l <= nl; ++l) hd[tid * hl + l] = 0.f;
    }
    dls[tid] = dl;
    dps[tid] = dp;
  }
  __syncthreads();
  __shared__ float cs[4][64];
  if (tid < kXeThreads - 256) {
    constexpr int NT = kXeThreads - 256;
    float* dst = xe + m0 * XE;
    const int n4 = nrows * XE >> 2;
    const float rxe = 1.f / (float)XE;
    for (int i4 = tid; i4 < n4; i4 += NT) {
      int rr = (int)(((float)(4 * i4) + 0.5f) * rxe);
      int c = 4 * i4 - rr * XE;
      float e[4];
#pragma unroll
      for (int u = 0; u < 4; ++u) {
        e[u] = c < F ? xs[rr * F + c] : c == F ? 1.f : c == F + 1 ? dls[rr] : dps[rr];
        if (++c == XE) {
          c = 0;
          ++rr;
        }
      }
      reinterpret_cast<float4*>(dst)[i4] = make_float4(e[0], e[1], e[2], e[3]);
    }
    for (int i = 4 * n4 + tid; i < nrows * XE; i += NT) {
      const int rr = i / XE, c = i - rr * XE;
      dst[i] = c < F ? xs[rr * F + c] : c == F ? 1.f : c == F + 1 ? dls[rr] : dps[rr];
    }
  } else {
    const int t2 = tid - (kXeThreads - 256);
    {
      const int f = t2 & 63, q = t2 >> 6;
      float t0 = 0.f, t1 = 0.f;
      if (f < F) {
        for (int rr = 64 * q; rr < 64 * q + 64; rr += 2) {
          t0 += xs[rr * F + f] * dls[rr];
          t1 += xs[(rr + 1) * F + f] * dls[rr + 1];
        }
      } else if (f < F + 2) {
        const float* dv = f == F ? dls : dps;
        for (int rr = 64 * q; rr < 64 * q + 64; rr += 2) {
          t0 += dv[rr];
          t1 += dv[rr + 1];
        }
      }
      cs[q][f] = t0 + t1;
    }
    if (g != nullptr) {
      const int k0 = (int)(m0 % K);
      for (int j = t2; j <= LK; j += 256) {
        float t = 0.f;
        if (j < LK) {
          const int l = j / K, k = j - l * K;
          for (int rr = (k - k0 + K) % K; rr < 256; rr += K) t += hd[rr * hl + l];
        } else {
          for (int rr = (K - k0) % K; rr < 256; rr += K) t += hd[rr * hl + nl];
        }
        hpart[(long)blockIdx.x * (LK + 1) + j] = t;
      }
    }
  }
  __syncthreads();
  if (tid < F + 2) dcpart[(long)blockIdx.x * kQtConst + tid] = (cs[0][tid] + cs[1][tid]) + (cs[2][tid] + cs[3][tid]);
}

constexpr int kDz2FieldStride = 128 * 2;
inline int cin_dz2_rows(int F, int JT) {
  const int hpp = cin_dz_h_per_period(JT);
  return std::max(cin_dz_sym_rows(F, JT), (F + hpp - 1) / hpp * hpp);
}

__device__ __forceinline__ void cin_dz2_finish(const float* smem, int wave, int lane, int wrow0, int M, int F, int K, const float* __restrict__ dsc, int ldp,
                                               float* __restrict__ dxT, int accumulate, float* __restrict__ dx, const float* __restrict__ cvec) {
  constexpr int FS = kDz2FieldStride;
  const float* img = smem + wave * 32 * 2 + 1;
  const int nrow = min(32, M - wrow0);
  if (dx != nullptr) {
    const int rr = lane & 31;
    const int mm = wrow0 + rr;
    const bool ok = rr < nrow;
    const long mc = ok ? mm : M - 1;
    const long bb = mc / K;
    const int kk = (int)(mc - bb * K);
    const float sc = dsc[bb * ldp + kk];
    float* dxb = dx + (bb * F) * K + kk;
    const float* add = dxT + mc * F;
    for (int f0 = lane >> 5; f0 < F; f0 += 16) {
      float a8[8];
#pragma unroll
      for (int u = 0; u < 8; ++u) a8[u] = accumulate ? add[min(f0 + 2 * u, F - 1)] : 0.f;
#pragma unroll
      for (int u = 0; u < 8; ++u) {
        const int f = f0 + 2 * u;
        if (f < F) {
          const float v = a8[u] + img[f * FS + rr * 2] + sc * cvec[f];
          if (ok) dxb[(long)f * K] = v;
        }
      }
    }
    return;
  }
  float* dst = dxT + (long)wrow0 * F;
  for (int idx = lane; idx < nrow * F; idx += 64) {
    const int rr = idx / F, f = idx - rr * F;
    const float v = img[f * FS + rr * 2];
    dst[idx] = accumulate ? dst[idx] + v : v;
  }
}

template <int JT, int G>
__global__ __launch_bounds__(256, 2) void cin_dz2_kernel(const float* __restrict__ g1T, const float* __restrict__ g2T, int HS,
                                                         const float* __restrict__ dsc, int ldp, int K, const float* __restrict__ Wz1,
                                                         const float* __restrict__ Wz2, const float* __restrict__ xT, float* __restrict__ dxT,
                                                         int accumulate, int M, int F, int H1, int H2, int periods, int FR,
                                                         float* __restrict__ dx, const float* __restrict__ cvec) {
  extern __shared__ __attribute__((aligned(16))) float smem[];
  constexpr int P = JT / gcd_c(16, JT);
  constexpr int HPP = 16 * P / JT;
  constexpr int NQ = 16;
  constexpr int FS = kDz2FieldStride;
  const int tid = threadIdx.x, lane = tid & 63, wave = tid >> 6;
  const int r = lane & 31, half = lane >> 5;
  const int wrow0 = (blockIdx.x * 4 + wave) * 32;
  if (wrow0 >= M) return;
  float* lrow = smem + (wave * 32 + r) * 2;
  const int m = wrow0 + r;
  const bool vq = m < M;
  const long mq = vq ? m : M - 1;
  f32x4s gq[16];
  {
    const f32x4s* grow4 = reinterpret_cast<const f32x4s*>(g1T + mq * HS + half * 64);
#pragma unroll
    for (int s4 = 0; s4 < 16; ++s4) gq[s4] = grow4[s4];
  }
  for (int f0 = half; f0 < FR; f0 += 16) {
    float xt[8];
#pragma unroll
    for (int u = 0; u < 8; ++u) xt[u] = xT[mq * F + min(f0 + 2 * u, F - 1)];
#pragma unroll
    for (int u = 0; u < 8; ++u) {
      const int f = f0 + 2 * u;
      if (f < FR) {
        const int keep = (vq && f < F) ? -1 : 0;
        *reinterpret_cast<float2*>(lrow + f * FS) = make_float2(__builtin_bit_cast(float, __builtin_bit_cast(int, xt[u]) & keep), 0.f);
      }
    }
  }
  float dpl;
  {
    const long bb = mq / K;
    dpl = dsc[bb * ldp + (mq - bb * K)];
  }
  __builtin_amdgcn_wave_barrier();
  const long wbytes = ((long)periods * P + 1) * 32 * 128 * 4;
  const int wo = (r * 128 + half * 64) * 4;
  float greg[64];
  auto to_greg = [&](const f32x4s (&gv4)[16], int Hk, float sc) {
#pragma unroll
    for (int s4 = 0; s4 < 16; ++s4)
#pragma unroll
      for (int e = 0; e < 4; ++e) {
        const int keep = (vq && half * 64 + 4 * s4 + e < Hk) ? -1 : 0;
        const float gv = gv4[s4][e];
        greg[4 * s4 + e] = __builtin_bit_cast(float, __builtin_bit_cast(int, gv) & keep) * sc;
      }
  };
  to_greg(gq, H1, 1.f);

#pragma unroll 1
  for (int pass = 0; pass < 2; ++pass) {
    const float* gT = pass == 0 ? g1T : g2T;
    const int Hk = pass == 0 ? H1 : H2;
    const float sc = pass == 0 ? 1.f : dpl;
    const __amdgpu_buffer_rsrc_t rw = make_rsrc(pass == 0 ? Wz1 : Wz2, wbytes);
    auto ldw = [&](int t, int s4) {
      return __builtin_bit_cast(f32x4s, __builtin_amdgcn_raw_buffer_load_b128(rw, wo + 16 * s4, t * (32 * 128 * 4), 0));
    };
    constexpr int QD = 8;
    f32x4s q[QD];
#pragma unroll
    for (int s4 = 0; s4 < QD; ++s4) q[s4] = ldw(0, s4);
    if (pass == 1) {
      const f32x4s* grow4 = reinterpret_cast<const f32x4s*>(gT + mq * HS + half * 64);
      f32x4s g2[16];
#pragma unroll
      for (int s4 = 0; s4 < 16; ++s4) g2[s4] = grow4[s4];
      to_greg(g2, Hk, sc);
    }
    float gx = 0.f;
    f32x16 dprev;
#pragma unroll
    for (int i = 0; i < 16; ++i) dprev[i] = 0.f;
    float xprev[HPP], xcur[HPP];
#pragma unroll
    for (int hl = 0; hl < HPP; ++hl) xprev[hl] = xcur[hl] = 0.f;
    int hprev = 0;
    float2 lv[G];
    float* la[G];
#pragma unroll
    for (int k = 0; k < G; ++k) {
      lv[k] = make_float2(0.f, 0.f);
      la[k] = lrow;
    }
    float *abase = lrow, *awrap = lrow;
    int symh = 0;
    auto sym_period = [&](int hb) {
      symh = hb + half;
      abase = lrow + symh * FS;
      awrap = abase - F * FS;
    };
    auto slot_fetch = [&](int tp, int rr, int k) {
      const int sp = 16 * tp + rr;
      const int off = sp / JT + 2 * (sp % JT);
      la[k] = (symh >= F - off ? awrap : abase) + off * FS;
      lv[k] = *reinterpret_cast<const float2*>(la[k]);
    };
    auto slot_apply = [&](const f32x16& d, const float (&xpv)[HPP], int hb, int tp, int rr, int k) {
      const int sp = 16 * tp + rr;
      const int hl = sp / JT, j = sp % JT;
      const float dz = d[rr];
      gx = fmaf(dz, lv[k].x, gx);
      la[k][1] = fmaf(dz, xpv[hl], lv[k].y);
      if (j == JT - 1) {
        const float t = lane_halves_sum(gx);
        gx = 0.f;
        if (half == 0) __hip_atomic_fetch_add(lrow + (hb + hl) * FS + 1, t, __ATOMIC_RELAXED, __HIP_MEMORY_SCOPE_WAVEFRONT);
      }
    };
    sym_period(hprev);
#pragma unroll
    for (int k = 0; k < G; ++k) slot_fetch(P - 1, k, k);
#pragma unroll 1
    for (int per = 0; per < periods; ++per) {
      const int hbase = per * HPP;
#pragma unroll
      for (int hl = 0; hl < HPP; ++hl) xcur[hl] = lrow[(hbase + hl) * FS];
#pragma unroll
      for (int tp = 0; tp < P; ++tp) {
        const int t = per * P + tp;
        f32x16 d;
#pragma unroll
        for (int i = 0; i < 16; ++i) d[i] = 0.f;
#pragma unroll
        for (int s4 = 0; s4 < NQ; ++s4) {
          const f32x4s w = q[s4 % QD];
          d = mfma32(w[0], greg[4 * s4 + 0], d);
          d = mfma32(w[1], greg[4 * s4 + 1], d);
          d = mfma32(w[2], greg[4 * s4 + 2], d);
          d = mfma32(w[3], greg[4 * s4 + 3], d);
          q[s4 % QD] = s4 + QD < NQ ? ldw(t, s4 + QD) : ldw(t + 1, s4 + QD - NQ);
          if (s4 % G == G - 1) {
#pragma unroll
            for (int k = 0; k < G; ++k) {
              const int rr = s4 - G + 1 + k;
              if (tp == 0) slot_apply(dprev, xprev, hprev, P - 1, rr, k);
              else slot_apply(dprev, xcur, hbase, tp - 1, rr, k);
            }
            if (s4 < 15) {
#pragma unroll
              for (int k = 0; k < G; ++k) slot_fetch(tp == 0 ? P - 1 : tp - 1, s4 + 1 + k, k);
            } else {
              if (tp == 0) sym_period(hbase);
#pragma unroll
              for (int k = 0; k < G; ++k) slot_fetch(tp, k, k);
            }
            __builtin_amdgcn_sched_barrier(0);
          }
        }
        dprev = d;
      }
#pragma unroll
      for (int hl = 0; hl < HPP; ++hl) xprev[hl] = xcur[hl];
      hprev = hbase;
    }
#pragma unroll
    for (int r0 = 0; r0 < 16; r0 += G) {
#pragma unroll
      for (int k = 0; k < G; ++k) slot_apply(dprev, xprev, hprev, P - 1, r0 + k, k);
      if (r0 + G < 16) {
#pragma unroll
        for (int k = 0; k < G; ++k) slot_fetch(P - 1, r0 + G + k, k);
      }
    }
  }
  __builtin_amdgcn_wave_barrier();
  cin_dz2_finish(smem, wave, lane, wrow0, M, F, K, dsc, ldp, dxT, accumulate, dx, cvec);
}

bool cin_launch_dz2(hipStream_t st, int JT, const float* g1T, const float* g2T, int HS, const float* dsc, int ldp, int K, const float* Wz1,
                    const float* Wz2, const float* xT, float* dxT, int accumulate, int M, int F, int H1, int H2, int periods,
                    float* dx = nullptr, const float* cvec = nullptr);

struct CinHeadFold {
  float* pooled;
  float* out;
  const float* dense_w;
  const float* dense_b;
  int kshift, LK, op, oL;
};

template <int NW>
__device__ __forceinline__ void cin_fwdq_epilogue(f32x16 (&acc)[8], const __amdgpu_buffer_rsrc_t& rx, int vhalf, int wo, int r, int half, int wave, int wrow0,
                                                  const float* __restrict__ bias1, const float* __restrict__ wsn, int JTG, const float* __restrict__ cvec,
                                                  float* __restrict__ x1T, float* __restrict__ RT, int HS, float* __restrict__ pool1,
                                                  float* __restrict__ pool_p, float* __restrict__ pool_L, int M, int F, int H, const CinHeadFold& hf,
                                                  float (&lin_s)[NW][32], float (&pv_s)[NW][3][32]) {
  const int lane = half * 32 + r;
  f32x16 t[4];
#pragma unroll
  for (int nb = 0; nb < 4; ++nb)
#pragma unroll
    for (int i = 0; i < 16; ++i) t[nb][i] = 0.f;
  const __amdgpu_buffer_rsrc_t rs = make_rsrc(wsn, (long)2 * JTG * 128 * 4);
  const __amdgpu_buffer_rsrc_t rc = make_rsrc(cvec, (long)kQtConst * 4);
  float xs4[2][4], cs4[2][4];
  f32x4s ws4[2][4];
  auto ldgroup = [&](int j0, int b) {
#pragma unroll
    for (int u = 0; u < 4; ++u) {
      const int j = __builtin_amdgcn_readfirstlane(j0) + u;
      xs4[b][u] = __builtin_bit_cast(float, __builtin_amdgcn_raw_buffer_load_b32(rx, vhalf, j * 512, 0));
      cs4[b][u] = __builtin_bit_cast(float, __builtin_amdgcn_raw_buffer_load_b32(rc, half * 4, j * 8, 0));
      ws4[b][u] = __builtin_bit_cast(f32x4s, __builtin_amdgcn_raw_buffer_load_b128(rs, wo, j * 1024, 0));
    }
  };
  float lin = 0.f;
  ldgroup(0, 0);
#pragma unroll 1
  for (int j0 = 0; j0 < JTG; j0 += 8) {
    ldgroup(j0 + 4, 1);
#pragma unroll
    for (int u = 0; u < 4; ++u) {
      const bool in = 2 * (j0 + u) + half < F;
      lin = fmaf(in ? xs4[0][u] : 0.f, in ? cs4[0][u] : 0.f, lin);
      const float a = xs4[0][u];
      t[0] = mfma32(a, ws4[0][u][0], t[0]);
      t[1] = mfma32(a, ws4[0][u][1], t[1]);
      t[2] = mfma32(a, ws4[0][u][2], t[2]);
      t[3] = mfma32(a, ws4[0][u][3], t[3]);
    }
    if (j0 + 4 < JTG) {
      ldgroup(j0 + 8, 0);
#pragma unroll
      for (int u = 0; u < 4; ++u) {
        const bool in = 2 * (j0 + 4 + u) + half < F;
        lin = fmaf(in ? xs4[1][u] : 0.f, in ? cs4[1][u] : 0.f, lin);
        const float a = xs4[1][u];
        t[0] = mfma32(a, ws4[1][u][0], t[0]);
        t[1] = mfma32(a, ws4[1][u][1], t[1]);
        t[2] = mfma32(a, ws4[1][u][2], t[2]);
        t[3] = mfma32(a, ws4[1][u][3], t[3]);
      }
    }
  }
  lin = lane_halves_sum(lin);
  if (half == 0) lin_s[wave][r] = lin;
  __builtin_amdgcn_wave_barrier();

  float bv[4];
#pragma unroll
  for (int nb = 0; nb < 4; ++nb) bv[nb] = 4 * r + nb < H ? bias1[4 * r + nb] : 0.f;
  const float cp = cvec[kQtConst + 1], cL = cvec[kQtConst];
#pragma unroll
  for (int reg = 0; reg < 16; ++reg) {
    const int row = mfma32_row(reg, half);
    const int m = wrow0 + row;
    const float a0 = acc[0][reg] + bv[0], a1 = acc[1][reg] + bv[1], a2 = acc[2][reg] + bv[2], a3 = acc[3][reg] + bv[3];
    const float b0 = acc[4][reg], b1 = acc[5][reg], b2 = acc[6][reg], b3 = acc[7][reg];
    if (m < M) {
      *reinterpret_cast<float4*>(x1T + (long)m * HS + 4 * r) = make_float4(a0, a1, a2, a3);
      *reinterpret_cast<float4*>(RT + (long)m * HS + 4 * r) = make_float4(b0, b1, b2, b3);
    }
    float p1 = (a0 + a1) + (a2 + a3);
    float eL = a0 * b0, ep = a0 * t[0][reg];
    eL = fmaf(a1, b1, eL);
    eL = fmaf(a2, b2, eL);
    eL = fmaf(a3, b3, eL);
    ep = fmaf(a1, t[1][reg], ep);
    ep = fmaf(a2, t[2][reg], ep);
    ep = fmaf(a3, t[3][reg], ep);
    p1 = half_wave_sum_hi(p1);
    eL = half_wave_sum_hi(eL);
    ep = half_wave_sum_hi(ep);
    if (r == 31 && m < M) {
      const float vp = ep + cp, vL = (eL + lin_s[wave][row]) + cL;
      if (hf.pooled != nullptr) {
        float* pr = hf.pooled + (long)(m >> hf.kshift) * hf.LK + (m & ((1 << hf.kshift) - 1));
        pr[0] = p1;
        pr[hf.op] = vp;
        pr[hf.oL] = vL;
        pv_s[wave][0][row] = p1;
        pv_s[wave][1][row] = vp;
        pv_s[wave][2][row] = vL;
      } else {
        pool1[m] = p1;
        pool_p[m] = vp;
        pool_L[m] = vL;
      }
    }
  }
  if (hf.out == nullptr) return;
  __builtin_amdgcn_wave_barrier();
  {
    const int k = (wrow0 + r) & ((1 << hf.kshift) - 1);
    const int o0 = half == 0 ? 0 : hf.op;
    pv_s[wave][half][r] *= hf.dense_w[o0 + k];
    if (half == 0) pv_s[wave][2][r] *= hf.dense_w[hf.oL + k];
  }
  __builtin_amdgcn_wave_barrier();
  const int K = 1 << hf.kshift;
  if (lane < (32 >> hf.kshift) && wrow0 + lane * K < M) {
    float o = 0.f;
    for (int l = 0; l < 3; ++l)
      for (int k = 0; k < K; ++k) o += pv_s[wave][l][lane * K + k];
    hf.out[(wrow0 >> hf.kshift) + lane] = o + hf.dense_b[0];
  }
}

template <int JT>
__global__ __launch_bounds__(256, 2) void cin_fwdq_kernel(const float* __restrict__ x2T, int XL, const float* __restrict__ W1f, const float* __restrict__ WTf,
                                                          const float* __restrict__ bias1, const float* __restrict__ wsn, int JTG,
                                                          const float* __restrict__ cvec, float* __restrict__ x1T, float* __restrict__ RT, int HS,
                                                          float* __restrict__ pool1, float* __restrict__ pool_p, float* __restrict__ pool_L, int M, int F,
                                                          int H, CinHeadFold hf) {
  constexpr int DEPTH = JT % 5 == 0 ? 5 : (JT % 4 == 0 ? 4 : (JT % 7 == 0 ? 7 : (JT % 3 == 0 ? 3 : 2)));
  static_assert(JT % DEPTH == 0, "queue depth must divide the steps per h");
  __shared__ float lin_s[4][32];
  __shared__ float pv_s[4][3][32];
  const int tid = threadIdx.x, lane = tid & 63, wave = tid >> 6;
  const int r = lane & 31, half = lane >> 5;
  const int wrow0 = (blockIdx.x * 4 + wave) * 32;
  if (wrow0 >= M) return;
  const int wrow_u = __builtin_amdgcn_readfirstlane(wrow0);
  const __amdgpu_buffer_rsrc_t rx = make_rsrc_uniform(x2T + (long)(wrow_u >> 6) * XL * 64, (long)XL * 256);
  const long wbytes = (long)F * (2 * JT) * 128 * 4;
  const __amdgpu_buffer_rsrc_t rw1 = make_rsrc(W1f, wbytes), rwt = make_rsrc(WTf, wbytes);
  const int wo = (half * 32 + r) * 16;
  const int vrow = ((wrow_u & 63) + r) * 4, vhalf = vrow + half * 256;
  auto ldw = [&](const __amdgpu_buffer_rsrc_t& rw, int s) {
    return __builtin_bit_cast(f32x4s, __builtin_amdgcn_raw_buffer_load_b128(rw, wo, s * 1024, 0));
  };
  auto ldfrag = [&](int h, float (&xf)[JT], float& xp) {
    const int hb = __builtin_amdgcn_readfirstlane(h) * 256;
    xp = __builtin_bit_cast(float, __builtin_amdgcn_raw_buffer_load_b32(rx, vrow, hb, 0));
#pragma unroll
    for (int j = 0; j < JT; ++j) xf[j] = __builtin_bit_cast(float, __builtin_amdgcn_raw_buffer_load_b32(rx, vhalf + 512 * j, hb, 0));
  };
  f32x16 acc[8];
#pragma unroll
  for (int nb = 0; nb < 8; ++nb)
#pragma unroll
    for (int i = 0; i < 16; ++i) acc[nb][i] = 0.f;
  f32x4s q1[DEPTH], qt[DEPTH];
#pragma unroll
  for (int d = 0; d < DEPTH; ++d) {
    q1[d] = ldw(rw1, d);
    qt[d] = ldw(rwt, d);
  }
  float xa[JT], xb[JT], pa, pb;
  ldfrag(0, xa, pa);
#pragma unroll
  for (int d = 0; d < DEPTH; ++d) {
    settle(q1[d]);
    settle(qt[d]);
  }
  settle(pa);
  float ac = pa * xa[0], an;
  auto run_h = [&](int h, float (&xc)[JT], float& pc, float (&xn_)[JT], float& pn) {
    ldfrag(min(h + 1, F - 1), xn_, pn);
    const int sb = h * JT;
#pragma unroll
    for (int j = 0; j < JT; ++j) {
      const f32x4s w1 = q1[j % DEPTH], wt = qt[j % DEPTH];
      an = j + 1 < JT ? pc * xc[j + 1 < JT ? j + 1 : 0] : pn * xn_[0];
      __builtin_amdgcn_sched_barrier(0);
      acc[0] = mfma32(ac, w1[0], acc[0]);
      acc[1] = mfma32(ac, w1[1], acc[1]);
      acc[2] = mfma32(ac, w1[2], acc[2]);
      acc[3] = mfma32(ac, w1[3], acc[3]);
      acc[4] = mfma32(ac, wt[0], acc[4]);
      acc[5] = mfma32(ac, wt[1], acc[5]);
      acc[6] = mfma32(ac, wt[2], acc[6]);
      acc[7] = mfma32(ac, wt[3], acc[7]);
      ac = an;
      __builtin_amdgcn_sched_barrier(0);
      q1[j % DEPTH] = ldw(rw1, sb + j + DEPTH);
      qt[j % DEPTH] = ldw(rwt, sb + j + DEPTH);
      __builtin_amdgcn_sched_barrier(0);
    }
  };
  int h = 0;
#pragma unroll 1
  for (; h + 1 < F; h += 2) {
    run_h(h, xa, pa, xb, pb);
    run_h(h + 1, xb, pb, xa, pa);
  }
  if (h < F) run_h(h, xa, pa, xb, pb);

  cin_fwdq_epilogue<4>(acc, rx, vhalf, wo, r, half, wave, wrow0, bias1, wsn, JTG, cvec, x1T, RT, HS, pool1, pool_p, pool_L, M, F, H, hf, lin_s, pv_s);
}

bool cin_launch_fwdq(hipStream_t st, int JT, const float* x2T, int XL, const float* W1f, const float* WTf, const float* bias1, const float* wsn, int JTG,
                     const float* cvec, float* x1T, float* RT, int HS, float* pool1, float* pool_p, float* pool_L, int M, int F, int H, CinHeadFold hf);

}
```

ml_function_amd/csrc/cin_qmerge.hip:

```cpp
#include "cin_qmerge.h"

namespace fil {

template <int JT, int G>
static void dz2g(hipStream_t st, const float* g1T, const float* g2T, int HS, const float* dsc, int ldp, int K, const float* Wz1, const float* Wz2,
                 const float* xT, float* dxT, int accumulate, int M, int F, int H1, int H2, int periods, float* dx, const float* cvec) {
  const int FR = cin_dz2_rows(F, JT);
  const size_t sh = (size_t)FR * kDz2FieldStride * sizeof(float);
  if (sh > 48 * 1024)
    (void)hipFuncSetAttribute(reinterpret_cast<const void*>(cin_dz2_kernel<JT, G>), hipFuncAttributeMaxDynamicSharedMemorySize, (int)sh);
  hipLaunchKernelGGL((cin_dz2_kernel<JT, G>), dim3(cdiv(M, 128)), dim3(kCinThreads), sh, st, g1T, g2T, HS, dsc, ldp, K, Wz1, Wz2, xT, dxT, accumulate, M, F, H1,
                     H2, periods, FR, dx, cvec);
}
template <int JT>
static void dz2(hipStream_t st, const float* g1T, const float* g2T, int HS, const float* dsc, int ldp, int K, const float* Wz1, const float* Wz2,
                const float* xT, float* dxT, int accumulate, int M, int F, int H1, int H2, int periods, float* dx, const float* cvec) {
  if (JT >= 4 && F >= cin_dz_h_per_period(JT) + 2 * JT) dz2g<JT, (JT >= 4 ? 4 : 1)>(st, g1T, g2T, HS, dsc, ldp, K, Wz1, Wz2, xT, dxT, accumulate, M, F, H1, H2, periods, dx, cvec);
  else dz2g<JT, 1>(st, g1T, g2T, HS, dsc, ldp, K, Wz1, Wz2, xT, dxT, accumulate, M, F, H1, H2, periods, dx, cvec);
}

bool cin_launch_dz2(hipStream_t st, int JT, const float* g1T, const float* g2T, int HS, const float* dsc, int ldp, int K, const float* Wz1,
                    const float* Wz2, const float* xT, float* dxT, int accumulate, int M, int F, int H1, int H2, int periods, float* dx, const float* cvec) {
#define FIL_Z2(JTV) \
  case JTV: dz2<JTV>(st, g1T, g2T, HS, dsc, ldp, K, Wz1, Wz2, xT, dxT, accumulate, M, F, H1, H2, periods, dx, cvec); break;
  switch (JT) { FIL_Z2(2) FIL_Z2(4) FIL_Z2(6) FIL_Z2(8) FIL_Z2(10) FIL_Z2(12) FIL_Z2(14) FIL_Z2(16) FIL_Z2(18) default: return false; }
#undef FIL_Z2
  return true;
}

bool cin_launch_fwdq(hipStream_t st, int JT, const float* x2T, int XL, const float* W1f, const float* WTf, const float* bias1, const float* wsn, int JTG,
                     const float* cvec, float* x1T, float* RT, int HS, float* pool1, float* pool_p, float* pool_L, int M, int F, int H, CinHeadFold hf) {
#define FIL_FQ(JTV)                                                                                                                             \
  case JTV:                                                                                                                                     \
    hipLaunchKernelGGL((cin_fwdq_kernel<JTV>), dim3(cdiv(M, 128)), dim3(kCinThreads), 0, st, x2T, XL, W1f, WTf, bias1, wsn, JTG, cvec, x1T, RT, HS, \
                       pool1, pool_p, pool_L, M, F, H, hf);                                                                                       \
    break;
  switch (JT) { FIL_FQ(2) FIL_FQ(4) FIL_FQ(6) FIL_FQ(8) FIL_FQ(10) FIL_FQ(12) FIL_FQ(14) FIL_FQ(16) FIL_FQ(18) default: return false; }
#undef FIL_FQ
  return true;
}

}
```

Baseline: 5.772 million.

## Fold head-gradient scaling of layer-1 gradient into forward epilogue and dW GEMM

Adds a gfold path for the output_dim==1 case. The forward epilogue now writes a per-sample head-weighted combination (wL*R + wp*T + w1) into RT in place of raw R. The backward then uses this precomputed buffer, scaled by the upstream gradient, instead of the layer-1 gradient produced by the last-bwd kernel. The last-bwd kernel therefore skips its T phase. The expanded xe matrix gains g-scaled x columns plus an extra ones column, so the dW GEMM also produces dbias1 and the separate bias reduction blocks are dropped. This removes a full M×HS gradient materialisation pass, at the cost of a wider xe and one extra GEMM column.

```diff
diff --git a/ml_function_amd/csrc/cin.hip b/ml_function_amd/csrc/cin.hip
--- a/ml_function_amd/csrc/cin.hip
+++ b/ml_function_amd/csrc/cin.hip
@@ -44,11 +44,11 @@
   return v != nullptr && *v != 0 ? atoi(v) : dflt;
 }
 struct Knobs {
-  int mb, sym, dw_mb, dw_splits, dz_mb, tail_splits, tail_settle, tail_dz_mode, ksplit, dzs_mb, qtail, qmerge, dz2, fwdq, headfold, packfold, dwfold4;
+  int mb, sym, dw_mb, dw_splits, dz_mb, tail_splits, tail_settle, tail_dz_mode, ksplit, dzs_mb, qtail, qmerge, dz2, fwdq, headfold, packfold, dwfold4, gfold;
 };
 static const Knobs& knobs() {
   static const Knobs k = {env_int("FIL_CIN_MB", 0), env_int("FIL_CIN_SYM", 1), env_int("FIL_CIN_DW_MB", 1), env_int("FIL_CIN_DW_SPLITS", 0),
-                          env_int("FIL_CIN_DZ_MB", 1), env_int("FIL_CIN_TAIL_SPLITS", 0), env_int("FIL_CIN_TAIL_SETTLE", 0), env_int("FIL_CIN_TAIL_DZ_MODE", 0), env_int("FIL_CIN_KSPLIT", -1), env_int("FIL_CIN_DZS_MB", 0), env_int("FIL_CIN_QTAIL", 1), env_int("FIL_CIN_QMERGE", 1), env_int("FIL_CIN_DZ2", 1), env_int("FIL_CIN_FWDQ", 1), env_int("FIL_CIN_HEADFOLD", 1), env_int("FIL_CIN_PACKFOLD", 1), env_int("FIL_CIN_DWFOLD4", 1)};
+                          env_int("FIL_CIN_DZ_MB", 1), env_int("FIL_CIN_TAIL_SPLITS", 0), env_int("FIL_CIN_TAIL_SETTLE", 0), env_int("FIL_CIN_TAIL_DZ_MODE", 0), env_int("FIL_CIN_KSPLIT", -1), env_int("FIL_CIN_DZS_MB", 0), env_int("FIL_CIN_QTAIL", 1), env_int("FIL_CIN_QMERGE", 1), env_int("FIL_CIN_DZ2", 1), env_int("FIL_CIN_FWDQ", 1), env_int("FIL_CIN_HEADFOLD", 1), env_int("FIL_CIN_PACKFOLD", 1), env_int("FIL_CIN_DWFOLD4", 1), env_int("FIL_CIN_GFOLD", 1)};
   return k;
 }
 struct CinTune {
@@ -190,6 +190,10 @@
   return (mode & (FIL_CIN_BF16X3 | kCinPrecBf16)) != 0 && qmerge_used(s, mode, tune) && knobs().fwdq != 0 && knobs().dz2 != 0 && s.HS(0) == 128 &&
          qsplit_fwd_menu(cin_jt_sym(s.F));
 }
+static bool gfold_used(const CinShape& s, int mode, const CinTune& tune, int output_dim) {
+  return output_dim == 1 && qmerge_used(s, mode, tune) && !qsplit_used(s, mode, tune) && knobs().fwdq != 0 && knobs().headfold != 0 &&
+         knobs().dz2 != 0 && s.HS(0) == 128 && s.K <= 32 && (s.K & (s.K - 1)) == 0 && knobs().gfold != 0;
+}
 static size_t qsplit_wb_bytes(const CinShape& s) { return (size_t)cin_qs_steps(s.F, cin_jt_sym(s.F)) * kQsStageBytes; }
 static size_t qsplit_wzb_bytes(const CinShape& s) {
   const int jts = cin_jt_sym(s.F);
@@ -275,7 +279,10 @@
   const int csym = s.F * (s.F / 2 + 1);
   pmax = std::max(pmax, (size_t)dw_plan(s.M(), csym, s.H[0]).splits * csym * s.H[0]);
   pmax = std::max(pmax, (size_t)dw_plan(s.M(), csym + s.F, s.H[0]).splits * (csym + s.F) * s.H[0]);
-  if (s.L == 3) pmax = std::max(pmax, (size_t)cin_dwq_plan(s.M(), csym + s.F, cu_count()).pairs * (csym + s.F) * 256);
+  for (int ones = 0; ones < 2 && s.L == 3; ++ones) {
+    const int cq = csym + s.F + ones;
+    pmax = std::max(pmax, (size_t)std::max(cin_dwq_plan(s.M(), cq, cu_count()).pairs, cin_dwq_plan4(s.M(), cq, cu_count()).pairs) * cq * 256);
+  }
   if (s.L == 3) pmax = std::max(pmax, (size_t)cin_dwqb_plan(s.M(), csym + s.F, cu_count()).splits * (csym + s.F) * 256);
   pmax = std::max(pmax, (size_t)dw_plan(s.M(), s.Hp(s.L - 1), s.F).splits * s.Hp(s.L - 1) * s.F);
   pmax = std::max(pmax, (size_t)dw_plan(s.M(), s.F, s.Hp(s.L - 1)).splits * s.Hp(s.L - 1) * s.F);
@@ -402,6 +409,7 @@
   const bool qmerge = qmerge_used(s, mode, tune);
   const bool qsplit = qsplit_used(s, mode, tune);
   const int qnp = qsplit_planes(mode);
+  const int mode_full = mode;
   const TailGeom tg = tail_geom(s);
   mode &= 1;
   if (B == 0) return FIL_OK;
@@ -524,7 +532,8 @@
         if (K <= 32 && (K & (K - 1)) == 0 && knobs().headfold != 0) {
           int ks = 0;
           while ((1 << ks) < K) ++ks;
-          hf = CinHeadFold{pooled, output_dim == 1 ? out : nullptr, dense_w, dense_b, ks, (int)(L * K), p * K, lL * K};
+          hf = CinHeadFold{pooled, output_dim == 1 ? out : nullptr, dense_w, dense_b, ks, (int)(L * K), p * K, lL * K,
+                           gfold_used(s, mode_full, tune, output_dim) ? 1 : 0};
           head_done = true;
         }
         if (qsplit) {
@@ -700,6 +709,7 @@
   const bool qmerge = qmerge_used(s, mode, tune);
   const bool qsplit = qsplit_used(s, mode, tune);
   const int qnp = qsplit_planes(mode);
+  const bool gfold = gfold_used(s, mode, tune, output_dim);
   const TailGeom tg = tail_geom(s);
   mode &= 1;
   FIL_CIN_CHECK_ARG(W && dW && dbias);
@@ -806,7 +816,7 @@
     const int JTs = cin_jt_sym(F);
     const int periods = cdiv(F, cin_dz_h_per_period(JTs));
     const int tiles0 = periods * cin_dz_tiles_per_period(JTs) + 1;
-    const int XE = F + 3;
+    const int XE = gfold ? 2 * F + 4 : F + 3;
     float* xe = Gbuf[1];
     float* gxR = xe + (size_t)M * XE;
     float* dxR = gxR + (size_t)M * F;
@@ -820,14 +830,18 @@
       if (qnp == 1)
         hipLaunchKernelGGL(cin_qtail_xe_kernel<1>, dim3(qt_ndc + np + nq2), dim3(kXeThreads), sh, st, xT, dPL, dPp, (int)LK, K, xe, qt_dcpart, (int)M, F,
                            qt_ndc, output_dim == 1 ? g : nullptr, dense_w, pooled, dP, qt_hpart, (int)LK, lL, p, W[0], Wz, H[0], JTs, HS0, tiles0, np, qtT,
-                           Hpp, Wzb1, Wzb2);
+                           Hpp, Wzb1, Wzb2, gfold ? 1 : 0);
       else
         hipLaunchKernelGGL(cin_qtail_xe_kernel<3>, dim3(qt_ndc + np + nq2), dim3(kXeThreads), sh, st, xT, dPL, dPp, (int)LK, K, xe, qt_dcpart, (int)M, F,
                            qt_ndc, output_dim == 1 ? g : nullptr, dense_w, pooled, dP, qt_hpart, (int)LK, lL, p, W[0], Wz, H[0], JTs, HS0, tiles0, np, qtT,
-                           Hpp, Wzb1, Wzb2);
-    }
-    FIL_CHECK_LAUNCH();
-    {
+                           Hpp, Wzb1, Wzb2, gfold ? 1 : 0);
+    }
+    FIL_CHECK_LAUNCH();
+    const float* g1src = gfold ? qtR : Gbuf[cur];
+    if (gfold) {
+      ProfScope ps("cin_last_bwd", st, 2.0 * (double)M * Hpp * F);
+      cin_launch_last_bwd2(st, JT, xT, xpT, xps, qtWsumP, qtWsnP, dPp, (int)LK, nullptr, nullptr, HS0, dxT, (int)M, F, K, Hpp);
+    } else {
       ProfScope ps("cin_last_bwd", st, 6.0 * (double)M * Hpp * F);
       cin_launch_last_bwd2(st, JT, xT, xpT, xps, qtWsumP, qtWsnP, dPp, (int)LK, dPprev, Gbuf[cur], HS0, dxT, (int)M, F, K, Hpp, qtR, HS0, dPL, small);
     }
@@ -841,12 +855,20 @@
         dw_parts = bp.splits;
       } else {
         const bool f4 = knobs().dwfold4 != 0;
-        const DwqPlan dp = f4 ? cin_dwq_plan4(M, Cl + F, cu_count()) : cin_dwq_plan(M, Cl + F, cu_count());
-        if (f4)
-          hipLaunchKernelGGL((cin_dwq_kernel<kDwqDepth, 4>), dim3((dp.wgs + 7) / 8 * 8), dim3(kDwqThreads), 0, st, Gbuf[cur], xpT, HS0, xe, XE, part, (int)M, F,
+        const int Cq = Cl + F + (gfold ? 1 : 0);
+        const DwqPlan dp = f4 ? cin_dwq_plan4(M, Cq, cu_count()) : cin_dwq_plan(M, Cq, cu_count());
+        const dim3 grid((dp.wgs + 7) / 8 * 8);
+        if (gfold && f4)
+          hipLaunchKernelGGL((cin_dwq_kernel<kDwqDepth, 4, true>), grid, dim3(kDwqThreads), 0, st, qtR, xpT, HS0, xe, XE, part, (int)M, F, symD, dp.rows_per_split,
+                             dp.splits, dp.ncol_full, dp.rem, dp.wgs_full, dp.wgs);
+        else if (gfold)
+          hipLaunchKernelGGL((cin_dwq_kernel<kDwqDepth, 2, true>), grid, dim3(kDwqThreads), 0, st, qtR, xpT, HS0, xe, XE, part, (int)M, F, symD, dp.rows_per_split,
+                             dp.splits, dp.ncol_full, dp.rem, dp.wgs_full, dp.wgs);
+        else if (f4)
+          hipLaunchKernelGGL((cin_dwq_kernel<kDwqDepth, 4>), grid, dim3(kDwqThreads), 0, st, Gbuf[cur], xpT, HS0, xe, XE, part, (int)M, F,
                              symD, dp.rows_per_split, dp.splits, dp.ncol_full, dp.rem, dp.wgs_full, dp.wgs);
         else
-          hipLaunchKernelGGL((cin_dwq_kernel<kDwqDepth, 2>), dim3((dp.wgs + 7) / 8 * 8), dim3(kDwqThreads), 0, st, Gbuf[cur], xpT, HS0, xe, XE, part, (int)M, F,
+          hipLaunchKernelGGL((cin_dwq_kernel<kDwqDepth, 2>), grid, dim3(kDwqThreads), 0, st, Gbuf[cur], xpT, HS0, xe, XE, part, (int)M, F,
                              symD, dp.rows_per_split, dp.splits, dp.ncol_full, dp.rem, dp.wgs_full, dp.wgs);
         dw_parts = dp.pairs;
       }
@@ -854,10 +876,11 @@
     FIL_CHECK_LAUNCH();
     {
       ProfScope ps("cin_reduce_dw", st);
-      const int nb1 = cdiv(H[0], 64);
+      const int ones = gfold ? 1 : 0;
+      const int nb1 = gfold ? 0 : cdiv(H[0], 64);
       const int nh = output_dim == 1 ? cdiv((int)LK + 1, 64) : 0;
-      hipLaunchKernelGGL(cin_reduce_expand_q_kernel, dim3((Cl + F + 3) / 4 + nb1 + nh), dim3(256), 0, st, part, dw_parts, F, symD, H[0], Hpp, dW[0], qt_dT,
-                         vlast, small, ncol, dbias[0], nb1, qt_hpart, qt_ndc, (int)LK, ddense_w, ddense_b);
+      hipLaunchKernelGGL(cin_reduce_expand_q_kernel, dim3((Cl + F + ones + 3) / 4 + nb1 + nh), dim3(256), 0, st, part, dw_parts, F, symD, H[0], Hpp, dW[0],
+                         qt_dT, vlast, small, ncol, dbias[0], nb1, qt_hpart, qt_ndc, (int)LK, ddense_w, ddense_b, ones);
     }
     FIL_CHECK_LAUNCH();
     ready(L);
@@ -883,7 +906,8 @@
         split_done = cin_launch_dz2_b(st, qnp, JTs, Gbuf[cur], xpT, HS0, dPL, (int)LK, K, Wzb1, Wzb2, xT, dxT, 1, (int)M, F, H[0], Hpp, periods, dx, qtCvec);
       }
       if (!split_done &&
-          !cin_launch_dz2(st, JTs, Gbuf[cur], xpT, HS0, dPL, (int)LK, K, Wz, qtWzT, xT, dxT, 1, (int)M, F, H[0], Hpp, periods, dx, qtCvec))
+          !cin_launch_dz2(st, JTs, g1src, xpT, HS0, dPL, (int)LK, K, Wz, qtWzT, xT, dxT, 1, (int)M, F, H[0], Hpp, periods, dx, qtCvec,
+                          gfold ? g : nullptr))
         return fail(FIL_ERR_UNSUPPORTED, "fil_cin_bwd: no two-pass data-gradient kernel for JT=%d (F=%d)", JTs, F);
       qm_joined = true;
     } else {
diff --git a/ml_function_amd/csrc/cin_kernels.h b/ml_function_amd/csrc/cin_kernels.h
--- a/ml_function_amd/csrc/cin_kernels.h
+++ b/ml_function_amd/csrc/cin_kernels.h
@@ -1282,7 +1282,7 @@
   const long mq = min(wrow0 + r, M - 1);
   float* stg = smem + ((Hp * F + 3) & ~3) + wave * kLast2Stage;
   const int nrow = min(32, M - wrow0);
-  if (nrow > 0) {
+  if (nrow > 0 && GprevT != nullptr) {
     const float4* src = reinterpret_cast<const float4*>(xT + (long)wrow0 * F);
     const int n4 = nrow * F / 4, tail = nrow * F - 4 * n4;
     for (int i = lane; i < n4; i += 64) *reinterpret_cast<float4*>(stg + 4 * i) = src[i];
@@ -1454,7 +1454,9 @@
     }
   }
   };
-  if ((blockIdx.x >> 3) & 1) {
+  if (GprevT == nullptr) {
+    phase_u();
+  } else if ((blockIdx.x >> 3) & 1) {
     phase_u();
     phase_t();
   } else {
diff --git a/ml_function_amd/csrc/cin_qmerge.h b/ml_function_amd/csrc/cin_qmerge.h
--- a/ml_function_amd/csrc/cin_qmerge.h
+++ b/ml_function_amd/csrc/cin_qmerge.h
@@ -54,14 +54,14 @@
   return p;
 }
 
-template <int DEPTH = kDwqDepth, int FOLD = 2>
+template <int DEPTH = kDwqDepth, int FOLD = 2, bool GS = false>
 __global__ __launch_bounds__(kDwqThreads, 2) void cin_dwq_kernel(const float* __restrict__ gT, const float* __restrict__ x1T, int HS, const float* __restrict__ xe,
                                                                 int XE, float* __restrict__ part, int M, int F, int symD, int rows_per_split, int splits,
                                                                 int ncol_full, int rem, int wgs_full, int wgs) {
   __shared__ float fold[4][128][64];
   const int tid = threadIdx.x, lane = tid & 63, wave = tid >> 6;
   const int r = lane & 31, half = lane >> 5;
-  const int Cp = F * symD, C = Cp + F;
+  const int Cp = F * symD, C = Cp + F + (GS ? 1 : 0);
   const int item = (blockIdx.x & 7) * (gridDim.x >> 3) + (blockIdx.x >> 3);
   if (item >= wgs) return;
   const int wl = FOLD == 4 ? (wave & 1) : (wave & 3), up = FOLD == 4 ? (wave >> 1) : (wave >> 2);
@@ -117,7 +117,7 @@
     ff = cc - Cp;
     sel = 1;
   }
-  const int ho = (half * XE + hh) * 4, fo = (half * XE + ff) * 4, so = (half * XE + F + 1 + sel) * 4;
+  const int ho = (half * XE + (GS ? F + 3 : 0) + hh) * 4, fo = (half * XE + ff) * 4, so = (half * XE + F + 1 + sel) * 4;
   const int go = (half * HS + 4 * r) * 4;
   const int steps = work ? (m_hi - m_lo + 1) >> 1 : 0;
   const int groups = (steps + DEPTH - 1) / DEPTH;
@@ -211,8 +211,8 @@
     const int cr = c0 + mfma32_row(reg, half);
     if (cr < C) {
       float* dst = pout + (long)cr * 256 + 4 * r;
-      if (cr < Cp) *reinterpret_cast<float4*>(dst) = make_float4(acc[0][reg], acc[1][reg], acc[2][reg], acc[3][reg]);
-      *reinterpret_cast<float4*>(dst + 128) = make_float4(acc[4][reg], acc[5][reg], acc[6][reg], acc[7][reg]);
+      if (cr < Cp || (GS && cr == C - 1)) *reinterpret_cast<float4*>(dst) = make_float4(acc[0][reg], acc[1][reg], acc[2][reg], acc[3][reg]);
+      if (!GS || cr < C - 1) *reinterpret_cast<float4*>(dst + 128) = make_float4(acc[4][reg], acc[5][reg], acc[6][reg], acc[7][reg]);
     }
   }
 }
@@ -221,8 +221,8 @@
                                                                           float* __restrict__ dW1, float* __restrict__ dT, float* __restrict__ vT,
                                                                           const float* __restrict__ bpart, int nbp, float* __restrict__ dbias1,
                                                                           int nb1, const float* __restrict__ hpart, int nhp, int LK,
-                                                                          float* __restrict__ ddw, float* __restrict__ ddb) {
-  const int Cp = F * D, C = Cp + F;
+                                                                          float* __restrict__ ddw, float* __restrict__ ddb, int ones = 0) {
+  const int Cp = F * D, C = Cp + F + ones;
   const int nbw = (C + 3) / 4;
   if ((int)blockIdx.x >= nbw + nb1) {
     cin_reduce_body(hpart, ddw, (long)LK + 1, nhp, ddb, (long)LK, (int)blockIdx.x - nbw - nb1);
@@ -250,6 +250,14 @@
   const int col = 4 * lane, n0 = col & 127;
   const bool second = col >= 128;
   const int H = second ? H2 : H1;
+  if (ones && c == C - 1) {
+    if (!second) {
+#pragma unroll
+      for (int e = 0; e < 4; ++e)
+        if (n0 + e < H1) dbias1[n0 + e] = v[e];
+    }
+    return;
+  }
   if (c >= Cp) {
     if (second) {
 #pragma unroll
@@ -287,7 +295,7 @@
                                                                   int LK, int lL, int lp, const float* __restrict__ W0, float* __restrict__ Wz,
                                                                   int H0, int JTs, int HS0, int tiles0, int npz = -1,
                                                                   const float* __restrict__ Tq = nullptr, int HT = 0, u32x4* __restrict__ Wzb1 = nullptr,
-                                                                  u32x4* __restrict__ Wzb2 = nullptr) {
+                                                                  u32x4* __restrict__ Wzb2 = nullptr, int gx = 0) {
   extern __shared__ __attribute__((aligned(16))) float smem[];
   if ((int)blockIdx.x >= nscale) {
     if (threadIdx.x >= 256) return;
@@ -302,7 +310,8 @@
     return;
   }
   const int nl = g != nullptr ? LK / K : 0;
-  const int hl = nl + 1, XE = F + 3;
+  const int hl = nl + 1, XE = gx ? 2 * F + 4 : F + 3;
+  __shared__ float gws[3][256];
   const int tid = threadIdx.x;
   const long m0 = (long)blockIdx.x * 256;
   const int nrows = (int)min((long)256, (long)M - m0);
@@ -345,6 +354,11 @@
         hd[tid * hl + nl] = k == 0 ? gb : 0.f;
         dl = gb * dense_w[lL * K + k];
         dp = gb * dense_w[lp * K + k];
+        if (gx) {
+          gws[0][tid] = gb;
+          gws[1][tid] = dense_w[lL * K + k];
+          gws[2][tid] = dense_w[lp * K + k];
+        }
       } else {
         dl = dPL[b * ldp + k];
         dp = dPp[b * ldp + k];
@@ -352,6 +366,7 @@
     } else if (g != nullptr) {
       for (int l = 0; l <= nl; ++l) hd[tid * hl + l] = 0.f;
     }
+    if (gx && m >= M) gws[0][tid] = gws[1][tid] = gws[2][tid] = 0.f;
     dls[tid] = dl;
     dps[tid] = dp;
   }
@@ -359,6 +374,13 @@
   __shared__ float cs[4][64];
   if (tid < kXeThreads - 256) {
     constexpr int NT = kXeThreads - 256;
+    auto elem = [&](int rr, int c) {
+      if (c < F) return xs[rr * F + c];
+      if (c == F) return 1.f;
+      if (c == F + 1) return gx ? gws[1][rr] : dls[rr];
+      if (c == F + 2) return gx ? gws[2][rr] : dps[rr];
+      return c < 2 * F + 3 ? gws[0][rr] * xs[rr * F + c - F - 3] : gws[0][rr];
+    };
     float* dst = xe + m0 * XE;
     const int n4 = nrows * XE >> 2;
     const float rxe = 1.f / (float)XE;
@@ -368,7 +390,7 @@
       float e[4];
 #pragma unroll
       for (int u = 0; u < 4; ++u) {
-        e[u] = c < F ? xs[rr * F + c] : c == F ? 1.f : c == F + 1 ? dls[rr] : dps[rr];
+        e[u] = elem(rr, c);
         if (++c == XE) {
           c = 0;
           ++rr;
@@ -378,7 +400,7 @@
     }
     for (int i = 4 * n4 + tid; i < nrows * XE; i += NT) {
       const int rr = i / XE, c = i - rr * XE;
-      dst[i] = c < F ? xs[rr * F + c] : c == F ? 1.f : c == F + 1 ? dls[rr] : dps[rr];
+      dst[i] = elem(rr, c);
     }
   } else {
     const int t2 = tid - (kXeThreads - 256);
@@ -466,7 +488,7 @@
                                                          const float* __restrict__ dsc, int ldp, int K, const float* __restrict__ Wz1,
                                                          const float* __restrict__ Wz2, const float* __restrict__ xT, float* __restrict__ dxT,
                                                          int accumulate, int M, int F, int H1, int H2, int periods, int FR,
-                                                         float* __restrict__ dx, const float* __restrict__ cvec) {
+                                                         float* __restrict__ dx, const float* __restrict__ cvec, const float* __restrict__ gs1) {
   extern __shared__ __attribute__((aligned(16))) float smem[];
   constexpr int P = JT / gcd_c(16, JT);
   constexpr int HPP = 16 * P / JT;
@@ -499,10 +521,11 @@
       }
     }
   }
-  float dpl;
+  float dpl, sc1 = 1.f;
   {
     const long bb = mq / K;
     dpl = dsc[bb * ldp + (mq - bb * K)];
+    if (gs1 != nullptr) sc1 = gs1[bb];
   }
   __builtin_amdgcn_wave_barrier();
   const long wbytes = ((long)periods * P + 1) * 32 * 128 * 4;
@@ -518,7 +541,7 @@
         greg[4 * s4 + e] = __builtin_bit_cast(float, __builtin_bit_cast(int, gv) & keep) * sc;
       }
   };
-  to_greg(gq, H1, 1.f);
+  to_greg(gq, H1, sc1);
 
 #pragma unroll 1
   for (int pass = 0; pass < 2; ++pass) {
@@ -642,7 +665,7 @@
 
 bool cin_launch_dz2(hipStream_t st, int JT, const float* g1T, const float* g2T, int HS, const float* dsc, int ldp, int K, const float* Wz1,
                     const float* Wz2, const float* xT, float* dxT, int accumulate, int M, int F, int H1, int H2, int periods,
-                    float* dx = nullptr, const float* cvec = nullptr);
+                    float* dx = nullptr, const float* cvec = nullptr, const float* gs1 = nullptr);
 
 struct CinHeadFold {
   float* pooled;
@@ -650,9 +673,10 @@
   const float* dense_w;
   const float* dense_b;
   int kshift, LK, op, oL;
+  int gfold;
 };
 
-template <int NW>
+template <int NW, bool GF = false>
 __device__ __forceinline__ void cin_fwdq_epilogue(f32x16 (&acc)[8], const __amdgpu_buffer_rsrc_t& rx, int vhalf, int wo, int r, int half, int wave, int wrow0,
                                                   const float* __restrict__ bias1, const float* __restrict__ wsn, int JTG, const float* __restrict__ cvec,
                                                   float* __restrict__ x1T, float* __restrict__ RT, int HS, float* __restrict__ pool1,
@@ -714,6 +738,20 @@
 #pragma unroll
   for (int nb = 0; nb < 4; ++nb) bv[nb] = 4 * r + nb < H ? bias1[4 * r + nb] : 0.f;
   const float cp = cvec[kQtConst + 1], cL = cvec[kQtConst];
+  __shared__ float hw_s[GF ? NW : 1][3][32];
+  const bool gf = GF && hf.gfold != 0;
+  float w1m[4];
+  if (gf) {
+    if (half == 0) {
+      const int k = r & ((1 << hf.kshift) - 1);
+      hw_s[wave][0][r] = hf.dense_w[hf.oL + k];
+      hw_s[wave][1][r] = hf.dense_w[hf.op + k];
+      hw_s[wave][2][r] = hf.dense_w[k];
+    }
+#pragma unroll
+    for (int nb = 0; nb < 4; ++nb) w1m[nb] = 4 * r + nb < H ? 1.f : 0.f;
+    __builtin_amdgcn_wave_barrier();
+  }
 #pragma unroll
   for (int reg = 0; reg < 16; ++reg) {
     const int row = mfma32_row(reg, half);
@@ -722,7 +760,14 @@
     const float b0 = acc[4][reg], b1 = acc[5][reg], b2 = acc[6][reg], b3 = acc[7][reg];
     if (m < M) {
       *reinterpret_cast<float4*>(x1T + (long)m * HS + 4 * r) = make_float4(a0, a1, a2, a3);
-      *reinterpret_cast<float4*>(RT + (long)m * HS + 4 * r) = make_float4(b0, b1, b2, b3);
+      if (gf) {
+        const float wL = hw_s[wave][0][row], wp = hw_s[wave][1][row], w1 = hw_s[wave][2][row];
+        *reinterpret_cast<float4*>(RT + (long)m * HS + 4 * r) =
+            make_float4(fmaf(wL, b0, fmaf(wp, t[0][reg], w1 * w1m[0])), fmaf(wL, b1, fmaf(wp, t[1][reg], w1 * w1m[1])),
+                        fmaf(wL, b2, fmaf(wp, t[2][reg], w1 * w1m[2])), fmaf(wL, b3, fmaf(wp, t[3][reg], w1 * w1m[3])));
+      } else {
+        *reinterpret_cast<float4*>(RT + (long)m * HS + 4 * r) = make_float4(b0, b1, b2, b3);
+      }
     }
     float p1 = (a0 + a1) + (a2 + a3);
     float eL = a0 * b0, ep = a0 * t[0][reg];
@@ -850,7 +895,7 @@
   }
   if (h < F) run_h(h, xa, pa, xb, pb);
 
-  cin_fwdq_epilogue<4>(acc, rx, vhalf, wo, r, half, wave, wrow0, bias1, wsn, JTG, cvec, x1T, RT, HS, pool1, pool_p, pool_L, M, F, H, hf, lin_s, pv_s);
+  cin_fwdq_epilogue<4, true>(acc, rx, vhalf, wo, r, half, wave, wrow0, bias1, wsn, JTG, cvec, x1T, RT, HS, pool1, pool_p, pool_L, M, F, H, hf, lin_s, pv_s);
 }
 
 bool cin_launch_fwdq(hipStream_t st, int JT, const float* x2T, int XL, const float* W1f, const float* WTf, const float* bias1, const float* wsn, int JTG,
diff --git a/ml_function_amd/csrc/cin_qmerge.hip b/ml_function_amd/csrc/cin_qmerge.hip
--- a/ml_function_amd/csrc/cin_qmerge.hip
+++ b/ml_function_amd/csrc/cin_qmerge.hip
@@ -4,25 +4,25 @@
 
 template <int JT, int G>
 static void dz2g(hipStream_t st, const float* g1T, const float* g2T, int HS, const float* dsc, int ldp, int K, const float* Wz1, const float* Wz2,
-                 const float* xT, float* dxT, int accumulate, int M, int F, int H1, int H2, int periods, float* dx, const float* cvec) {
+                 const float* xT, float* dxT, int accumulate, int M, int F, int H1, int H2, int periods, float* dx, const float* cvec, const float* gs1) {
   const int FR = cin_dz2_rows(F, JT);
   const size_t sh = (size_t)FR * kDz2FieldStride * sizeof(float);
   if (sh > 48 * 1024)
     (void)hipFuncSetAttribute(reinterpret_cast<const void*>(cin_dz2_kernel<JT, G>), hipFuncAttributeMaxDynamicSharedMemorySize, (int)sh);
   hipLaunchKernelGGL((cin_dz2_kernel<JT, G>), dim3(cdiv(M, 128)), dim3(kCinThreads), sh, st, g1T, g2T, HS, dsc, ldp, K, Wz1, Wz2, xT, dxT, accumulate, M, F, H1,
-                     H2, periods, FR, dx, cvec);
+                     H2, periods, FR, dx, cvec, gs1);
 }
 template <int JT>
 static void dz2(hipStream_t st, const float* g1T, const float* g2T, int HS, const float* dsc, int ldp, int K, const float* Wz1, const float* Wz2,
-                const float* xT, float* dxT, int accumulate, int M, int F, int H1, int H2, int periods, float* dx, const float* cvec) {
-  if (JT >= 4 && F >= cin_dz_h_per_period(JT) + 2 * JT) dz2g<JT, (JT >= 4 ? 4 : 1)>(st, g1T, g2T, HS, dsc, ldp, K, Wz1, Wz2, xT, dxT, accumulate, M, F, H1, H2, periods, dx, cvec);
-  else dz2g<JT, 1>(st, g1T, g2T, HS, dsc, ldp, K, Wz1, Wz2, xT, dxT, accumulate, M, F, H1, H2, periods, dx, cvec);
+                const float* xT, float* dxT, int accumulate, int M, int F, int H1, int H2, int periods, float* dx, const float* cvec, const float* gs1) {
+  if (JT >= 4 && F >= cin_dz_h_per_period(JT) + 2 * JT) dz2g<JT, (JT >= 4 ? 4 : 1)>(st, g1T, g2T, HS, dsc, ldp, K, Wz1, Wz2, xT, dxT, accumulate, M, F, H1, H2, periods, dx, cvec, gs1);
+  else dz2g<JT, 1>(st, g1T, g2T, HS, dsc, ldp, K, Wz1, Wz2, xT, dxT, accumulate, M, F, H1, H2, periods, dx, cvec, gs1);
 }
 
 bool cin_launch_dz2(hipStream_t st, int JT, const float* g1T, const float* g2T, int HS, const float* dsc, int ldp, int K, const float* Wz1,
-                    const float* Wz2, const float* xT, float* dxT, int accumulate, int M, int F, int H1, int H2, int periods, float* dx, const float* cvec) {
+                    const float* Wz2, const float* xT, float* dxT, int accumulate, int M, int F, int H1, int H2, int periods, float* dx, const float* cvec, const float* gs1) {
 #define FIL_Z2(JTV) \
-  case JTV: dz2<JTV>(st, g1T, g2T, HS, dsc, ldp, K, Wz1, Wz2, xT, dxT, accumulate, M, F, H1, H2, periods, dx, cvec); break;
+  case JTV: dz2<JTV>(st, g1T, g2T, HS, dsc, ldp, K, Wz1, Wz2, xT, dxT, accumulate, M, F, H1, H2, periods, dx, cvec, gs1); break;
   switch (JT) { FIL_Z2(2) FIL_Z2(4) FIL_Z2(6) FIL_Z2(8) FIL_Z2(10) FIL_Z2(12) FIL_Z2(14) FIL_Z2(16) FIL_Z2(18) default: return false; }
 #undef FIL_Z2
   return true;
```

Measured after the change: 5.839 million, median of 6. 1.01x the previous value.
